# r9y9/nnmnkwii

Measured on AMD Instinct MI355X. Metric: MLPG frames/sec (batch, 60-dim mgc x3 windows), higher is better.
Workload: dtype f64

## Files before the change

nnmnkwii_amd/csrc/mlpg_strip.hip:

```cpp
#include <map>
#include <mutex>
#include <utility>
#include <limits.h>
#include <string.h>

#include "common.h"

namespace mlpg {

int launch_strip_fwd_f64(hipStream_t st, int out_dtype, const Problem &p, const WinSet &ws, void *scratch, int R, int ndg, int dgw, bool zero_ctrl);
int launch_strip_fwd_f32(hipStream_t st, int out_dtype, const Problem &p, const WinSet &ws, void *scratch, int R, int ndg, int dgw, bool zero_ctrl);
int launch_strip_bwd_f64(hipStream_t st, int out_dtype, const Problem &p, const WinSet &ws, void *scratch, int R, int ndg, int dgw, bool zero_ctrl);
int launch_strip_bwd_f32(hipStream_t st, int out_dtype, const Problem &p, const WinSet &ws, void *scratch, int R, int ndg, int dgw, bool zero_ctrl);
int launch_strip_multi_f64(hipStream_t st, const Problem &p, const WinSet &ws, void *scratch, int R, int ndg, int dgw, bool zero_ctrl, const StreamMap &sm);
int launch_strip_multi_f32(hipStream_t st, const Problem &p, const WinSet &ws, void *scratch, int R, int ndg, int dgw, bool zero_ctrl, const StreamMap &sm);
int launch_strip_tr_f64(hipStream_t st, const Problem &p, const WinSet &ws, void *scratch, int R, bool zero_ctrl, const StreamMap &sm);
int launch_strip_tr_f32(hipStream_t st, const Problem &p, const WinSet &ws, void *scratch, int R, bool zero_ctrl, const StreamMap &sm);

namespace {
#ifndef MLPG_STRIP_W
#define MLPG_STRIP_W 4
#endif
#ifndef MLPG_STRIP_M
#define MLPG_STRIP_M 16
#endif
constexpr int kStripFrames = MLPG_STRIP_M * MLPG_STRIP_W;
constexpr int kMaxStrips = 256;
constexpr int kRecBytes = 14 * 64 * 8;
constexpr int kStripNotResident = kStripMultiNotResident;
}

bool strip_supported(const Problem &p, const WinSet &ws) {
  if (p.Tmax < 1 || (p.Tmax + kStripFrames - 1) / kStripFrames > kMaxStrips) return false;
  for (int w = 0; w < ws.nw; ++w)
    if (ws.l[w] > 1 || ws.u[w] > 1) return false;
  return rows_fit_buffer(p);
}

bool strip_preferred(const Problem &p, const WinSet &ws, bool backward, int in_dtype) {
  if (!strip_supported(p, ws)) return false;
  if (p.sd >= 16 && p.Tmax > 1024) return true;
  const int ndg = (p.sd + 63) / 64, dgw = (p.sd + ndg - 1) / ndg;
  const long nitems = (long)p.B * ndg * ((p.Tmax + kStripFrames - 1) / kStripFrames);
  if (dgw < 48) return false;
  if (p.var_mode != MLPG_HIP_VAR_FRAME) return false;
  (void)backward;
  (void)in_dtype;
  return nitems >= 512;
}

bool strip_tr_supported(const Problem &p, const WinSet &ws, bool backward, int in_dtype, int out_dtype) {
  if (backward || in_dtype != out_dtype || ws.nw != 3) return false;
  if (p.sd < 1 || p.sd > 32 || p.B < 2 || !strip_supported(p, ws)) return false;
  const int u = 64 / p.sd;
  const long ld = p.ld_in > p.ld_out ? p.ld_in : p.ld_out;
  return (double)u * (double)p.Tmax * (double)ld * 8.0 < 2147483647.0;
}
bool strip_tr_preferred(const Problem &p, const WinSet &ws, bool backward, int in_dtype, int out_dtype) {
  if (!strip_tr_supported(p, ws, backward, in_dtype, out_dtype)) return false;
  const int u = 64 / p.sd;
  const long items = (long)((p.B + u - 1) / u) * ((p.Tmax + kStripFrames - 1) / kStripFrames);
  if (p.B < u) return false;
  if (p.Tmax > 1024) return items >= 64;
  return items >= (in_dtype == MLPG_HIP_F32 ? 512 : 256);
}

namespace {
std::mutex g_clean_mu;
std::map<std::pair<int, hipStream_t>, std::pair<unsigned long long, size_t>> g_clean;
void strip_scratch_forget(hipStream_t st, int device) {
  std::lock_guard<std::mutex> lk(g_clean_mu);
  g_clean[{device, st}].second = 0;
}
void *strip_scratch(hipStream_t st, int device, size_t nsg, int R, bool *zero_ctrl) {
  const size_t ctrl = (((1 + 16 + nsg) * 32 + nsg * (size_t)((R + 31) / 32 * 32)) * sizeof(int) + 255) / 256 * 256;
  unsigned long long gen = 0;
  void *sc = scratch(device, st, 3, ctrl + nsg * R * kRecBytes, &gen);
  if (!sc) return nullptr;
  *zero_ctrl = true;
  hipStreamCaptureStatus cap = hipStreamCaptureStatusNone;
  const bool capturing = hipStreamIsCapturing(st, &cap) != hipSuccess || cap != hipStreamCaptureStatusNone;
  std::lock_guard<std::mutex> lk(g_clean_mu);
  auto &c = g_clean[{device, st}];
  if (!capturing && c.first == gen && ctrl <= c.second) *zero_ctrl = false;
  c = {gen, capturing ? (size_t)0 : ctrl};
  return sc;
}
}

namespace {
__global__ void xcc_probe_kernel(int *hist) {
  if (threadIdx.x == 0) atomicAdd_system(hist + (__builtin_amdgcn_s_getreg((3 << 11) | (0 << 6) | 20) & 7), 1);
}
}
bool strip_xcd_lists_ok(hipStream_t st) {
  static std::mutex mu;
  static std::map<int, bool> seen;
  static std::map<int, int> failed;
  int dev = 0;
  if (hipGetDevice(&dev) != hipSuccess) return false;
  std::lock_guard<std::mutex> lk(mu);
  auto it = seen.find(dev);
  if (it != seen.end()) return it->second;
  hipStreamCaptureStatus cap = hipStreamCaptureStatusNone;
  if (hipStreamIsCapturing(st, &cap) != hipSuccess || cap != hipStreamCaptureStatusNone) {
    (void)hipGetLastError();
    return false;
  }
  hipStreamCaptureMode mode = hipStreamCaptureModeRelaxed;
  const bool mode_set = hipThreadExchangeStreamCaptureMode(&mode) == hipSuccess;
  bool ok = false, probed = false;
  int *h = nullptr;
  hipStream_t ps = nullptr;
  constexpr int kBlocks = 4096;
  if (hipHostMalloc((void **)&h, 8 * sizeof(int), hipHostMallocDefault) == hipSuccess) {
    for (int k = 0; k < 8; ++k) h[k] = 0;
    if (hipStreamCreateWithFlags(&ps, hipStreamNonBlocking) == hipSuccess) {
      hipLaunchKernelGGL(xcc_probe_kernel, dim3(kBlocks), dim3(64), 0, ps, h);
      if (hipGetLastError() == hipSuccess && hipStreamSynchronize(ps) == hipSuccess) {
        int lo = h[0], hi = h[0];
        for (int k = 1; k < 8; ++k) { lo = h[k] < lo ? h[k] : lo; hi = h[k] > hi ? h[k] : hi; }
        ok = lo > 0 && 2 * lo >= hi;
        probed = true;
      }
      (void)hipStreamDestroy(ps);
    }
    (void)hipHostFree(h);
  }
  (void)hipGetLastError();
  if (mode_set) (void)hipThreadExchangeStreamCaptureMode(&mode);
  if (probed) seen[dev] = ok;
  else if (++failed[dev] >= 3) seen[dev] = false;
  return ok;
}

int launch_strip_tr(hipStream_t st, int dtype, const Problem &p, const WinSet &ws, int device) {
  const int R = (p.Tmax + kStripFrames - 1) / kStripFrames;
  StreamMap sm;
  memset(&sm, 0, sizeof(sm));
  for (int q = 0; q < 4; ++q) sm.begin[q] = INT_MAX;
  sm.n = 1;
  sm.begin[0] = 0;
  sm.sd[0] = p.pitch ? p.pitch : p.sd;
  sm.tr_nd = p.sd;
  sm.tr_u = 64 / p.sd;
  sm.total = sm.tr_u * sm.tr_nd;
  sm.tr_B = p.B;
  sm.tr_in = (int)((long)p.Tmax * p.ld_in);
  sm.tr_out = (int)((long)p.Tmax * p.ld_out);
  sm.tr_stat = p.ld_status;
  const size_t nsg = (size_t)(p.B + sm.tr_u - 1) / sm.tr_u;
  bool zero_ctrl = true;
  void *sc = strip_scratch(st, device, nsg, R, &zero_ctrl);
  if (!sc) return MLPG_HIP_ENOMEM;
  const int rc = dtype == MLPG_HIP_F32 ? launch_strip_tr_f32(st, p, ws, sc, R, zero_ctrl, sm) : launch_strip_tr_f64(st, p, ws, sc, R, zero_ctrl, sm);
  if (rc == kStripNotResident) strip_scratch_forget(st, device);
  return rc;
}

int launch_strip(hipStream_t st, int dtype, int out_dtype, bool backward, const Problem &p, const WinSet &ws,
                 int device, bool try_tr) {
  if (try_tr && strip_tr_supported(p, ws, backward, dtype, out_dtype)) {
    const int rc = launch_strip_tr(st, dtype, p, ws, device);
    if (rc != kStripNotResident) return rc;
  }
  const int R = (p.Tmax + kStripFrames - 1) / kStripFrames;
  const int ndg = (p.sd + 63) / 64;
  const int dgw = (p.sd + ndg - 1) / ndg;
  const size_t nsg = (size_t)p.B * ndg;
  bool zero_ctrl = true;
  void *sc = strip_scratch(st, device, nsg, R, &zero_ctrl);
  if (!sc) return MLPG_HIP_ENOMEM;
  int rc;
  if (!backward)
    rc = dtype == MLPG_HIP_F32 ? launch_strip_fwd_f32(st, out_dtype, p, ws, sc, R, ndg, dgw, zero_ctrl)
                               : launch_strip_fwd_f64(st, out_dtype, p, ws, sc, R, ndg, dgw, zero_ctrl);
  else
    rc = dtype == MLPG_HIP_F32 ? launch_strip_bwd_f32(st, out_dtype, p, ws, sc, R, ndg, dgw, zero_ctrl)
                               : launch_strip_bwd_f64(st, out_dtype, p, ws, sc, R, ndg, dgw, zero_ctrl);
  if (rc == kStripNotResident) {
    strip_scratch_forget(st, device);
    return launch_generic(st, dtype, out_dtype, backward, p, ws, device);
  }
  return rc;
}

int launch_strip_multi(hipStream_t st, int dtype, const Problem &p, const WinSet &ws, const StreamMap &sm, int device) {
  const int R = (p.Tmax + kStripFrames - 1) / kStripFrames;
  const int ndg = (sm.total + 63) / 64;
  const int dgw = 64;
  const size_t nsg = (size_t)p.B * ndg;
  bool zero_ctrl = true;
  void *sc = strip_scratch(st, device, nsg, R, &zero_ctrl);
  if (!sc) return MLPG_HIP_ENOMEM;
  const int rc = dtype == MLPG_HIP_F32 ? launch_strip_multi_f32(st, p, ws, sc, R, ndg, dgw, zero_ctrl, sm)
                                       : launch_strip_multi_f64(st, p, ws, sc, R, ndg, dgw, zero_ctrl, sm);
  if (rc == kStripNotResident) strip_scratch_forget(st, device);
  return rc;
}

}
```

nnmnkwii_amd/csrc/mlpg_strip_bwd_f32.hip:

```cpp
#include "mlpg_strip_impl.h"
namespace mlpg {
int launch_strip_bwd_f32(hipStream_t st, int out_dtype, const Problem &p, const WinSet &ws, void *scratch, int R, int ndg, int dgw, bool zero_ctrl) {
  if (out_dtype == MLPG_HIP_F32) return strip::launch_t<float, float, true>(st, p, ws, scratch, R, ndg, dgw, zero_ctrl);
  return strip::launch_t<float, double, true>(st, p, ws, scratch, R, ndg, dgw, zero_ctrl);
}
}
```

nnmnkwii_amd/csrc/mlpg_strip_bwd_f64.hip:

```cpp
#include "mlpg_strip_impl.h"
namespace mlpg {
int launch_strip_bwd_f64(hipStream_t st, int out_dtype, const Problem &p, const WinSet &ws, void *scratch, int R, int ndg, int dgw, bool zero_ctrl) {
  if (out_dtype == MLPG_HIP_F32) return strip::launch_t<double, float, true>(st, p, ws, scratch, R, ndg, dgw, zero_ctrl);
  return strip::launch_t<double, double, true>(st, p, ws, scratch, R, ndg, dgw, zero_ctrl);
}
}
```

nnmnkwii_amd/csrc/mlpg_strip_fwd_f32.hip:

```cpp
#include "mlpg_strip_impl.h"
namespace mlpg {
int launch_strip_fwd_f32(hipStream_t st, int out_dtype, const Problem &p, const WinSet &ws, void *scratch, int R, int ndg, int dgw, bool zero_ctrl) {
  (void)out_dtype;
  return strip::launch_t<float, float, false>(st, p, ws, scratch, R, ndg, dgw, zero_ctrl);
}
}
```

nnmnkwii_amd/csrc/mlpg_strip_fwd_f64.hip:

```cpp
#include "mlpg_strip_impl.h"
namespace mlpg {
int launch_strip_fwd_f64(hipStream_t st, int out_dtype, const Problem &p, const WinSet &ws, void *scratch, int R, int ndg, int dgw, bool zero_ctrl) {
  (void)out_dtype;
  return strip::launch_t<double, double, false>(st, p, ws, scratch, R, ndg, dgw, zero_ctrl);
}
}
```

nnmnkwii_amd/csrc/mlpg_strip_impl.h:

```cpp
#pragma once
#include <stdlib.h>
#include <string.h>

#include <type_traits>

#include <mutex>
#include <vector>
#include "assemble.h"

#ifndef MLPG_STRIP_ABLATE
#define MLPG_STRIP_ABLATE 0
#endif
#ifdef MLPG_STRIP_TIMING
#define STRIP_TICK(k)                                                  \
  do {                                                                 \
    const long long t_now_ = (long long)__builtin_readcyclecounter(); \
    tq[k] += t_now_ - t_prev;                                          \
    t_prev = t_now_;                                                   \
  } while (0)
#else
#define STRIP_TICK(k) do {} while (0)
#endif

namespace mlpg {
namespace strip {

#ifndef MLPG_STRIP_W
#define MLPG_STRIP_W 4
#endif
#ifndef MLPG_STRIP_M
#define MLPG_STRIP_M 16
#endif
#ifndef MLPG_STRIP_WGS
#define MLPG_STRIP_WGS (MLPG_STRIP_W <= 4 ? 2 : 1)
#endif
constexpr int kW = MLPG_STRIP_W;
constexpr int kM = MLPG_STRIP_M;
constexpr int kN = kM - 2;
constexpr int kRec = 14;
#ifndef MLPG_STRIP_DAMP1_TOL
#define MLPG_STRIP_DAMP1_TOL 0x1p-66
#endif
#ifndef MLPG_STRIP_STAGE
#define MLPG_STRIP_STAGE (MLPG_STRIP_W > 6 ? 8 : 6)
#endif
constexpr int kStage = MLPG_STRIP_STAGE;
constexpr bool kParkOn = kM >= 16;
constexpr int kPark = kParkOn ? 2 * kN : 0;
constexpr int kFac = 10;
constexpr int kSpinLimit = 1 << 20;

enum { rT00, rT01, rT11, rH0, rH1, rD11, rD12, rD22, rF1, rF2, rL11, rL12, rL21, rL22 };

constexpr int kCtrlLine = 32;
#ifndef MLPG_STRIP_POLL_SLEEP
#define MLPG_STRIP_POLL_SLEEP 16
#endif
#ifndef MLPG_STRIP_RING_F32
#define MLPG_STRIP_RING_F32 6
#endif
#ifndef MLPG_STRIP_BWD_FRAME_MAJOR
#define MLPG_STRIP_BWD_FRAME_MAJOR 1
#endif
#ifndef MLPG_STRIP_BWD_KEEP
#define MLPG_STRIP_BWD_KEEP 1
#endif
#ifndef MLPG_STRIP_FWD_BUFSTORE
#define MLPG_STRIP_FWD_BUFSTORE 1
#endif
#ifndef MLPG_STRIP_BWD_BUFSTORE
#define MLPG_STRIP_BWD_BUFSTORE 1
#endif
#ifndef MLPG_STRIP_BWD_KARG
#define MLPG_STRIP_BWD_KARG 1
#endif
#ifndef MLPG_STRIP_FWD_KARG
#define MLPG_STRIP_FWD_KARG 1
#endif
#ifndef MLPG_STRIP_BWD_KEEP0
#define MLPG_STRIP_BWD_KEEP0 1
#endif
#ifndef MLPG_STRIP_BWD_EARLY0
#define MLPG_STRIP_BWD_EARLY0 0
#endif
#ifndef MLPG_STRIP_BWD_EARLY
#define MLPG_STRIP_BWD_EARLY 4
#endif
#ifndef MLPG_STRIP_NT_STORES
#define MLPG_STRIP_NT_STORES 1
#endif
#ifndef MLPG_STRIP_RING_F64
#define MLPG_STRIP_RING_F64 6
#endif
#ifndef MLPG_STRIP_STAGGER_DEFAULT_US
#define MLPG_STRIP_STAGGER_DEFAULT_US 0
#endif

#ifndef MLPG_STRIP_ROUTE1_TOL
#define MLPG_STRIP_ROUTE1_TOL 0x1p-66
#endif
constexpr int kMaxLists = 8;
constexpr int kLocal = 2;
constexpr double kRouteTol = 1e-11;
constexpr double kDampTol = 1e-22;
constexpr double kDamp1Tol = MLPG_STRIP_DAMP1_TOL;
struct Window { int lo, hiE, edge; };
__device__ __forceinline__ Window local_window(int r, int Ract, int k) {
  Window w;
  w.lo = r - k < 0 ? 0 : r - k;
  w.edge = r + k < Ract - 1;
  w.hiE = w.edge ? r + k : Ract - 1;
  return w;
}
struct Order { int lo, hiE, r, nt, nb, m, npos; };
__device__ __forceinline__ Order make_order(int r, int lo, int hiE) {
  Order o;
  o.lo = lo; o.hiE = hiE; o.r = r;
  o.nt = r - lo;
  o.nb = hiE - r;
  o.m = o.nt < o.nb ? o.nt : o.nb;
  o.npos = o.nt + o.nb + 1;
  return o;
}
__device__ __forceinline__ int row_of(const Order &o, int pos) {
  if (pos < 2 * o.m) return (pos & 1) ? o.hiE - (pos >> 1) : o.lo + (pos >> 1);
  if (pos < o.nt + o.nb) {
    const int k = o.m + (pos - 2 * o.m);
    return o.nt > o.nb ? o.lo + k : o.hiE - k;
  }
  return o.r;
}
__host__ __device__ inline int flag_pitch(int R) { return (R + kCtrlLine - 1) / kCtrlLine * kCtrlLine; }
__host__ __device__ inline size_t ctrl_ints(int nsg, int R) {
  return (size_t)(1 + kMaxLists + nsg) * kCtrlLine + (size_t)nsg * flag_pitch(R);
}

struct Args {
  int *ctrl;
  double *rec;
  int R;
  int ndg, dgw;
  int nsg;
  double one;
  double wc[kMaxWindows][9];
  int nlists;
  int nb, bs;
  StreamMap sm;
  int stagger;
  int wpl;
};

template <bool MULTI = false>
__device__ __forceinline__ void ticket_item(const Args &a, int tk, int lst, int &g, int &r) {
  if (MULTI) {
    g = (((tk / a.R) / a.ndg) * a.nlists + lst) * a.ndg + (tk / a.R) % a.ndg;
    r = tk % a.R;
  } else {
    const int v = (tk / a.bs) * a.nlists + lst;
    g = v / a.nb;
    r = (v - g * a.nb) * a.bs + tk % a.bs;
  }
}

struct LaneStream { int sd, din, dstat, dout, dvar; };
__device__ __forceinline__ LaneStream lane_stream_tr(const StreamMap &sm, int d) {
  const int u = d / sm.tr_nd, dl = d - u * sm.tr_nd;
  return {sm.sd[0], u * sm.tr_in + sm.in_col[0] + dl, u * sm.tr_stat + sm.stat_col[0] + dl, u * sm.tr_out + sm.out_col[0] + dl,
          sm.in_col[0] + dl};
}
__device__ __forceinline__ LaneStream lane_stream(const StreamMap &sm, int d) {
  const int s_ = (d >= sm.begin[1]) + (d >= sm.begin[2]) + (d >= sm.begin[3]);
  auto pick = [&](const int (&v)[4]) { return s_ == 0 ? v[0] : s_ == 1 ? v[1] : s_ == 2 ? v[2] : v[3]; };
  const int dl = d - pick(sm.begin);
  return {pick(sm.sd), dl + pick(sm.in_col), dl + pick(sm.stat_col), dl + pick(sm.out_col), dl + pick(sm.in_col)};
}

constexpr size_t kLdsStage = (size_t)kStage * kRec * 64 * 8;
constexpr size_t kLdsPark = (size_t)kPark * 64 * 8;
constexpr size_t kLdsFac = (size_t)(kW - 1) * kFac * 64 * 8;
constexpr size_t kLdsU = (size_t)(kW + 1) * 2 * 64 * 8;
constexpr size_t kLdsMisc = 64 + kW * 256;
constexpr size_t kLdsBytes = kLdsStage + kLdsPark + kLdsFac + kLdsU + kLdsMisc;
static_assert(kW * kRec <= kStage * kRec, "level-1 records must fit the staging area");
static_assert(kLdsBytes <= 160 * 1024 / MLPG_STRIP_WGS, "MLPG_STRIP_WGS workgroups per CU must fit the 160 KB of LDS");

__device__ __forceinline__ double fast_rcp(double d) {
  double x = __builtin_amdgcn_rcp(d);
  x = __builtin_fma(__builtin_fma(-d, x, 1.0), x, x);
  x = __builtin_fma(__builtin_fma(-d, x, 1.0), x, x);
  return x;
}
template <typename T>
__device__ __forceinline__ double tau_of(T v);
template <>
__device__ __forceinline__ double tau_of<float>(float v) {
  return (double)__fdiv_rn(1.0f, v);
}
template <>
__device__ __forceinline__ double tau_of<double>(double v) {
  return fast_rcp(v);
}

struct S2 { double a, b, c; };
struct M2 { double a, b, c, d; };
struct V2 { double x, y; };

__device__ __forceinline__ S2 sym_inv(const S2 &E, bool &bad) {
  const double det = E.a * E.c - E.b * E.b;
  bad |= (E.a <= 0.0) | (det <= 0.0) | !(det == det);
  const double idet = fast_rcp(det);
  return {E.c * idet, -E.b * idet, E.a * idet};
}
__device__ __forceinline__ M2 mul_ms(const M2 &L, const S2 &S) {
  return {L.a * S.a + L.b * S.b, L.a * S.b + L.b * S.c, L.c * S.a + L.d * S.b, L.c * S.b + L.d * S.c};
}
__device__ __forceinline__ M2 mul_sm(const S2 &S, const M2 &V) {
  return {S.a * V.a + S.b * V.c, S.a * V.b + S.b * V.d, S.b * V.a + S.c * V.c, S.b * V.b + S.c * V.d};
}
__device__ __forceinline__ M2 mul_smt(const S2 &S, const M2 &V) {
  return {S.a * V.a + S.b * V.b, S.a * V.c + S.b * V.d, S.b * V.a + S.c * V.b, S.b * V.c + S.c * V.d};
}
__device__ __forceinline__ double amax4(const M2 &m) {
  return __builtin_fmax(__builtin_fmax(__builtin_fabs(m.a), __builtin_fabs(m.b)),
                        __builtin_fmax(__builtin_fabs(m.c), __builtin_fabs(m.d)));
}
__device__ __forceinline__ M2 mul_mm(const M2 &A, const M2 &B) {
  return {A.a * B.a + A.b * B.c, A.a * B.b + A.b * B.d, A.c * B.a + A.d * B.c, A.c * B.b + A.d * B.d};
}
__device__ __forceinline__ S2 mul_mmt_sym(const M2 &A, const M2 &B) {
  return {A.a * B.a + A.b * B.b, A.a * B.c + A.b * B.d, A.c * B.c + A.d * B.d};
}
__device__ __forceinline__ S2 mul_mtm_sym(const M2 &A, const M2 &B) {
  return {A.a * B.a + A.c * B.c, A.a * B.b + A.c * B.d, A.b * B.b + A.d * B.d};
}
__device__ __forceinline__ V2 mul_mv(const M2 &A, const V2 &v) { return {A.a * v.x + A.b * v.y, A.c * v.x + A.d * v.y}; }
__device__ __forceinline__ V2 mul_mtv(const M2 &A, const V2 &v) { return {A.a * v.x + A.c * v.y, A.b * v.x + A.d * v.y}; }
__device__ __forceinline__ V2 mul_sv(const S2 &S, const V2 &v) { return {S.a * v.x + S.b * v.y, S.b * v.x + S.c * v.y}; }
__device__ __forceinline__ S2 sub(const S2 &A, const S2 &B) { return {A.a - B.a, A.b - B.b, A.c - B.c}; }
__device__ __forceinline__ S2 add(const S2 &A, const S2 &B) { return {A.a + B.a, A.b + B.b, A.c + B.c}; }
__device__ __forceinline__ V2 sub(const V2 &A, const V2 &B) { return {A.x - B.x, A.y - B.y}; }
__device__ __forceinline__ V2 add(const V2 &A, const V2 &B) { return {A.x + B.x, A.y + B.y}; }
__device__ __forceinline__ M2 neg(const M2 &A) { return {-A.a, -A.b, -A.c, -A.d}; }
__device__ __forceinline__ M2 transpose(const M2 &A) { return {A.a, A.c, A.b, A.d}; }

__device__ __forceinline__ void st_agent(double *p, double v) {
  __hip_atomic_store((unsigned long long *)p, (unsigned long long)__double_as_longlong(v), __ATOMIC_RELAXED,
                     __HIP_MEMORY_SCOPE_AGENT);
}
__device__ __forceinline__ double ld_agent(const double *p) {
  return __longlong_as_double((long long)__hip_atomic_load((const unsigned long long *)p, __ATOMIC_RELAXED,
                                                           __HIP_MEMORY_SCOPE_AGENT));
}

constexpr int kNB = kM == 16 ? 6 : 2;
constexpr int kHB = (kM + 2) / kNB;
static_assert(kHB * kNB == kM + 2, "batches must tile the 18 frames");

typedef __attribute__((ext_vector_type(2))) unsigned int u32x2;
template <typename TIN>
__device__ __forceinline__ TIN ld_row(__amdgpu_buffer_rsrc_t rs, unsigned soff, unsigned loff);
template <>
__device__ __forceinline__ double ld_row<double>(__amdgpu_buffer_rsrc_t rs, unsigned soff, unsigned loff) {
  const u32x2 v = __builtin_amdgcn_raw_buffer_load_b64(rs, loff, soff, 0);
  return __longlong_as_double((long long)(((unsigned long long)v.y << 32) | v.x));
}
template <>
__device__ __forceinline__ float ld_row<float>(__amdgpu_buffer_rsrc_t rs, unsigned soff, unsigned loff) {
  return __uint_as_float(__builtin_amdgcn_raw_buffer_load_b32(rs, loff, soff, 0));
}
template <typename TIN>
__device__ __forceinline__ TIN ld_row_g(__amdgpu_buffer_rsrc_t rs, unsigned soff, unsigned loff);
template <>
__device__ __forceinline__ double ld_row_g<double>(__amdgpu_buffer_rsrc_t rs, unsigned soff, unsigned loff) {
  const u32x2 v = __builtin_amdgcn_raw_buffer_load_b64(rs, loff, soff, 0);
  return __longlong_as_double((long long)(((unsigned long long)v.y << 32) | v.x));
}
template <>
__device__ __forceinline__ float ld_row_g<float>(__amdgpu_buffer_rsrc_t rs, unsigned soff, unsigned loff) {
  return __uint_as_float(__builtin_amdgcn_raw_buffer_load_b32(rs, loff, soff, 0));
}
__device__ __forceinline__ __amdgpu_buffer_rsrc_t make_rsrc(const void *base) {
  const unsigned long long u = (unsigned long long)base;
  const unsigned lo = __builtin_amdgcn_readfirstlane((unsigned)u), hi = __builtin_amdgcn_readfirstlane((unsigned)(u >> 32));
  return __builtin_amdgcn_make_buffer_rsrc((void *)(((unsigned long long)hi << 32) | lo), 0, 0x7fffffff, 0x00020000);
}

__device__ __forceinline__ void st_row(__amdgpu_buffer_rsrc_t rs, unsigned soff, unsigned loff, double v) {
  const unsigned long long u = (unsigned long long)__double_as_longlong(v);
  const u32x2 w = {(unsigned)u, (unsigned)(u >> 32)};
  __builtin_amdgcn_raw_buffer_store_b64(w, rs, loff, soff, MLPG_STRIP_NT_STORES ? 2 : 0);
}
__device__ __forceinline__ void st_row(__amdgpu_buffer_rsrc_t rs, unsigned soff, unsigned loff, float v) {
  __builtin_amdgcn_raw_buffer_store_b32(__float_as_uint(v), rs, loff, soff, MLPG_STRIP_NT_STORES ? 2 : 0);
}

typedef __attribute__((ext_vector_type(8))) unsigned u32x8;
typedef __attribute__((ext_vector_type(4))) unsigned u32x4;
__device__ __forceinline__ double mk_f64(unsigned lo, unsigned hi) {
  return __longlong_as_double((long long)(((unsigned long long)hi << 32) | lo));
}
template <unsigned OFF>
__device__ __forceinline__ void karg_f64x6(double (&d)[6]) {
  const unsigned long long kp = (unsigned long long)__builtin_amdgcn_kernarg_segment_ptr();
  u32x8 a;
  u32x4 b;
  asm volatile("s_load_dwordx8 %0, %2, %3\n\ts_load_dwordx4 %1, %2, %4\n\ts_waitcnt lgkmcnt(0)"
               : "=&s"(a), "=&s"(b)
               : "s"(kp), "n"(OFF), "n"(OFF + 32));
  d[0] = mk_f64(a[0], a[1]); d[1] = mk_f64(a[2], a[3]); d[2] = mk_f64(a[4], a[5]); d[3] = mk_f64(a[6], a[7]);
  d[4] = mk_f64(b[0], b[1]); d[5] = mk_f64(b[2], b[3]);
}
typedef __attribute__((ext_vector_type(16))) unsigned u32x16;
template <unsigned OFF>
__device__ __forceinline__ void karg_f64x9(double (&d)[9]) {
  const unsigned long long kp = (unsigned long long)__builtin_amdgcn_kernarg_segment_ptr();
  u32x16 a;
  u32x2 b;
  asm volatile("s_load_dwordx16 %0, %2, %3\n\ts_load_dwordx2 %1, %2, %4\n\ts_waitcnt lgkmcnt(0)"
               : "=&s"(a), "=&s"(b)
               : "s"(kp), "n"(OFF), "n"(OFF + 64));
#pragma unroll
  for (int q = 0; q < 8; ++q) d[q] = mk_f64(a[2 * q], a[2 * q + 1]);
  d[8] = mk_f64(b[0], b[1]);
}
template <unsigned OFF>
__device__ __forceinline__ void karg_f64x3(double (&d)[3]) {
  const unsigned long long kp = (unsigned long long)__builtin_amdgcn_kernarg_segment_ptr();
  u32x4 a;
  u32x2 b;
  asm volatile("s_load_dwordx4 %0, %2, %3\n\ts_load_dwordx2 %1, %2, %4\n\ts_waitcnt lgkmcnt(0)"
               : "=&s"(a), "=&s"(b)
               : "s"(kp), "n"(OFF), "n"(OFF + 16));
  d[0] = mk_f64(a[0], a[1]); d[1] = mk_f64(a[2], a[3]); d[2] = mk_f64(b[0], b[1]);
}
constexpr unsigned kKargWs = (unsigned)((sizeof(Problem) + alignof(WinSet) - 1) / alignof(WinSet) * alignof(WinSet));
constexpr unsigned kKargArgs = (unsigned)((kKargWs + sizeof(WinSet) + alignof(Args) - 1) / alignof(Args) * alignof(Args));
constexpr unsigned kKargWc = kKargArgs + (unsigned)__builtin_offsetof(Args, wc);

template <typename TIN, bool BWD, int VM, bool EDGE, int H>
__device__ __forceinline__ void load_batch(TIN (&rv)[kHB], TIN (&rm)[kHB], __amdgpu_buffer_rsrc_t mrs,
                                           __amdgpu_buffer_rsrc_t vrs, unsigned woff, unsigned loff, unsigned ldi_bytes,
                                           int f0, int lo, int hi) {
#pragma unroll
  for (int q = 0; q < kHB; ++q) {
    int t = f0 + H * kHB + q - 1;
    if (EDGE) t = t < lo ? lo : (t >= hi ? hi - 1 : t);
    const unsigned soff = (unsigned)t * ldi_bytes + woff;
    if (VM == MLPG_HIP_VAR_FRAME) rv[q] = ld_row<TIN>(vrs, soff, loff);
    if (!BWD) rm[q] = ld_row<TIN>(mrs, soff, loff);
  }
}

struct WinCoef {
  double cm, c0, cp, c00, cpp, cmm, cp0, c0m, cpm, tau_glob;
  int w;
};

template <typename TIN, bool BWD, int VM, bool EDGE, int H>
__device__ __forceinline__ void accumulate(const TIN (&rv)[kHB], const TIN (&rm)[kHB], const WinCoef &k, int f0, int lo,
                                           int hi, double (&Pd)[kM], double (&P1)[kM], double (&P2)[kM],
                                           double (&rhs)[kM], double &ca, double &cb, double &cc) {
#pragma unroll
  for (int q = 0; q < kHB; ++q) {
    const int i = H * kHB + q - 1;
    const int t = f0 + i;
    double tau = VM == MLPG_HIP_VAR_FRAME ? tau_of<TIN>(rv[q]) : k.tau_glob;
    if (MLPG_STRIP_ABLATE >= 3) {
      if (i >= 0 && i < kM) { Pd[i] += VM == MLPG_HIP_VAR_FRAME ? (double)rv[q] : 1.0; if (!BWD) rhs[i] += (double)rm[q]; }
      continue;
    }
    if (EDGE) tau *= (t >= lo && t < hi) ? 1.0 : 0.0;
    double tm = 0.0;
    if (!BWD) tm = tau * (double)rm[q];
    if (i >= 0 && i < kM) {
      Pd[i] += k.c00 * tau;
      P1[i] += k.cp0 * tau;
      if (!BWD) rhs[i] += k.c0 * tm;
    }
    if (i + 1 >= 0 && i + 1 < kM) {
      Pd[i + 1] += k.cpp * tau;
      if (!BWD) rhs[i + 1] += k.cp * tm;
    }
    if (i - 1 >= 0 && i - 1 < kM) {
      Pd[i - 1] += k.cmm * tau;
      P1[i - 1] += k.c0m * tau;
      P2[i - 1] += k.cpm * tau;
      if (!BWD) rhs[i - 1] += k.cm * tm;
    }
    if (i == -1) {
      ca += k.cpm * tau;
      cb += k.cp0 * tau;
    }
    if (i == 0) {
      cb += k.c0m * tau;
      cc += k.cpm * tau;
    }
  }
}

template <typename TIN, int VM>
__device__ __forceinline__ WinCoef win_coef(const double (*wc)[9], int w, const TIN *vglob, int sd) {
  WinCoef k;
  k.cm = wc[w][0]; k.c0 = wc[w][1]; k.cp = wc[w][2];
  k.c00 = wc[w][3]; k.cpp = wc[w][4]; k.cmm = wc[w][5];
  k.cp0 = wc[w][6]; k.c0m = wc[w][7]; k.cpm = wc[w][8];
  k.tau_glob = 1.0;
  if (VM == MLPG_HIP_VAR_GLOBAL) k.tau_glob = tau_of<TIN>(vglob[w * sd]);
  k.w = w;
  return k;
}

template <typename TIN, bool BWD, int VM, bool EDGE>
__device__ __forceinline__ void assemble(__amdgpu_buffer_rsrc_t mrs, __amdgpu_buffer_rsrc_t vrs,
                                         __amdgpu_buffer_rsrc_t grs, const TIN *__restrict__ vglob, unsigned loff,
                                         long ldi, long ldg, int sd, int f0, int T, int Tmax, const WinSet &ws,
                                         const double (*wc)[9], double (&Pd)[kM], double (&P1)[kM], double (&P2)[kM], double (&rhs)[kM],
                                         double &ca, double &cb, double &cc) {
#pragma unroll
  for (int i = 0; i < kM; ++i) Pd[i] = P1[i] = P2[i] = rhs[i] = 0.0;
  ca = cb = cc = 0.0;
  const int mw = ws.mw, nw = ws.nw;
  const unsigned ldi_bytes = (unsigned)ldi * (unsigned)sizeof(TIN), win_bytes = (unsigned)sd * (unsigned)sizeof(TIN);
  auto live_lo = [&](int w) { return w ? mw : 0; };
  auto live_hi = [&](int w) { return w ? (mw != 0 && T - mw > mw ? T - mw : mw) : T; };
  TIN rvA[kHB], rmA[kHB], rvB[kHB], rmB[kHB];
  auto clo = [&](int w) { const int l_ = live_lo(w); return l_ < T ? l_ : T - 1; };
  auto chi = [&](int w) { const int h_ = live_hi(w), l_ = clo(w); return h_ > l_ ? h_ : l_ + 1; };
  load_batch<TIN, BWD, VM, EDGE, 0>(rvA, rmA, mrs, vrs, 0u, loff, ldi_bytes, f0, clo(0), chi(0));
  if (BWD) {
#pragma unroll
    for (int i = 0; i < kM; ++i) {
      int t = f0 + i;
      if (EDGE) t = t >= T ? T - 1 : t;
      rhs[i] = (double)ld_row_g<TIN>(grs, (unsigned)t * (unsigned)ldg * (unsigned)sizeof(TIN), loff);
    }
  }
  for (int w = 0; w < nw; ++w) {
    const WinCoef k = win_coef<TIN, VM>(wc, w, vglob, sd);
    const unsigned woff = (unsigned)w * win_bytes;
    const int lo = live_lo(w), hi = live_hi(w), cl = clo(w), ch = chi(w);
#define STRIP_STEP(H, RVX, RMX, RVY, RMY)                                                                      \
    if ((H) + 1 < kNB) {                                                                                          \
    load_batch<TIN, BWD, VM, EDGE, ((H) + 1 < kNB ? (H) + 1 : 0)>(RVY, RMY, mrs, vrs, woff, loff, ldi_bytes, f0, cl, ch);             \
    __builtin_amdgcn_sched_barrier(0);                                                                          \
    accumulate<TIN, BWD, VM, EDGE, (H)>(RVX, RMX, k, f0, lo, hi, Pd, P1, P2, rhs, ca, cb, cc);                  \
    __builtin_amdgcn_sched_barrier(0);                                                                          \
    }
    STRIP_STEP(0, rvA, rmA, rvB, rmB)
    STRIP_STEP(1, rvB, rmB, rvA, rmA)
    STRIP_STEP(2, rvA, rmA, rvB, rmB)
    STRIP_STEP(3, rvB, rmB, rvA, rmA)
    STRIP_STEP(4, rvA, rmA, rvB, rmB)
#undef STRIP_STEP
    if (w + 1 < nw) load_batch<TIN, BWD, VM, EDGE, 0>(rvA, rmA, mrs, vrs, woff + win_bytes, loff, ldi_bytes, f0, clo(w + 1), chi(w + 1));
    __builtin_amdgcn_sched_barrier(0);
    accumulate<TIN, BWD, VM, EDGE, kNB - 1>(rvB, rmB, k, f0, lo, hi, Pd, P1, P2, rhs, ca, cb, cc);
    __builtin_amdgcn_sched_barrier(0);
  }
  if (EDGE) {
#pragma unroll
    for (int i = 0; i < kM; ++i) {
      const int f = f0 + i;
      if (f >= T) {
        Pd[i] = 1.0;
        P1[i] = P2[i] = rhs[i] = 0.0;
      } else {
        if (f + 1 >= T) P1[i] = 0.0;
        if (f + 2 >= T) P2[i] = 0.0;
      }
    }
    if (f0 == 0 || f0 >= T) ca = cb = cc = 0.0;
    else if (f0 + 1 >= T) cc = 0.0;
  }
}

__device__ __forceinline__ bool eliminate(double (&Pd)[kM], double (&P1)[kM], double (&P2)[kM], double (&rhs)[kM],
                                          double ca, double cb, double cc, double (&rec)[kRec]) {
  bool bad = false;
  double t00 = 0.0, t01 = 0.0, t11 = 0.0, h0 = 0.0, h1 = 0.0;
  double g1 = 0.0, g2 = 0.0, va1 = 0.0, va2 = 0.0, vb1 = 0.0, vb2 = 0.0;
  double l1p = 0.0, l2p = 0.0, l2pp = 0.0;
#pragma unroll
  for (int i = 0; i < kN; ++i) {
    const double dd = Pd[i];
    bad |= !(dd > 0.0);
    const double dinv = fast_rcp(dd);
    const double e1 = P1[i], e2 = P2[i];
    const double l1 = e1 * dinv, l2 = e2 * dinv;
    Pd[i + 1] -= l1 * e1;
    P1[i + 1] -= l2 * e1;
    Pd[i + 2] -= l2 * e2;
    const double gi = rhs[i] - l1p * g1 - l2pp * g2;
    const double ba = (i == 0) ? ca : 0.0;
    const double bb = (i == 0) ? cb : ((i == 1) ? cc : 0.0);
    const double va = ba - l1p * va1 - l2pp * va2;
    const double vb = bb - l1p * vb1 - l2pp * vb2;
    const double wa = va * dinv, wb = vb * dinv;
    t00 += wa * va;
    t01 += wa * vb;
    t11 += wb * vb;
    h0 += wa * gi;
    h1 += wb * gi;
    Pd[i] = dinv;
    P1[i] = l1;
    P2[i] = l2;
    rhs[i] = gi;
    g2 = g1; g1 = gi;
    va2 = va1; va1 = va;
    vb2 = vb1; vb1 = vb;
    l2pp = l2p; l2p = l2; l1p = l1;
    __builtin_amdgcn_sched_barrier(0);
  }
  rec[rT00] = t00; rec[rT01] = t01; rec[rT11] = t11; rec[rH0] = h0; rec[rH1] = h1;
  rec[rD11] = Pd[kN]; rec[rD12] = P1[kN]; rec[rD22] = Pd[kN + 1];
  rec[rF1] = rhs[kN] - (l1p * g1 + l2pp * g2);
  rec[rF2] = rhs[kN + 1] - l2p * g1;
  rec[rL11] = -(l1p * va1 + l2pp * va2);
  rec[rL12] = -(l1p * vb1 + l2pp * vb2);
  rec[rL21] = -(l2p * va1);
  rec[rL22] = -(l2p * vb1);
  return bad;
}

constexpr int kStd4[3][9] = {{0, 4, 0, 4, 0, 0, 0, 0, 0}, {-2, 0, 2, 0, 1, 1, 0, 0, -1}, {4, -8, 4, 16, 4, 4, -8, -8, 4}};
enum { qCm, qC0, qCp, qC00, qCpp, qCmm, qCp0, qC0m, qCpm };
constexpr int std_first(int q) { return kStd4[0][q] ? 0 : (kStd4[1][q] ? 1 : 2); }
constexpr bool std_last_has_all() {
  for (int q = 0; q < 9; ++q)
    if (kStd4[2][q] == 0) return false;
  return true;
}
static_assert(std_last_has_all(), "every entry has a window that contributes (std_first)");
__device__ __forceinline__ void std_term(double &acc, const int w, const int q, const double x, const bool init) {
  const int c4 = kStd4[w][q];
  if (c4 == 0) return;
  if (init && w == std_first(q)) acc = c4 == 4 ? x : (c4 == -4 ? -x : (0.25 * c4) * x);
  else acc = c4 == 4 ? acc + x : (c4 == -4 ? acc - x : __builtin_fma(0.25 * c4, x, acc));
}
__device__ __forceinline__ double std_apply(const int w, const double xm, const double x0, const double xp) {
  if (w == 0) return x0;
  if (w == 1) return __builtin_fma(0.5, xp, -0.5 * xm);
  return __builtin_fma(-2.0, x0, xm) + xp;
}
inline bool std_windows(const WinSet &ws, const double (*wc)[9]) {
  if (ws.nw != 3 || ws.l[0] != 0 || ws.u[0] != 0 || ws.l[1] != 1 || ws.u[1] != 1 || ws.l[2] != 1 || ws.u[2] != 1) return false;
  for (int w = 0; w < 3; ++w)
    for (int q = 0; q < 9; ++q)
      if (!(wc[w][q] == 0.25 * kStd4[w][q])) return false;
  return true;
}
inline bool stdwin_enabled() {
  static const bool on = [] { const char *e = getenv("MLPG_STRIP_STDWIN"); return !(e && *e && atoi(e) == 0); }();
  return on;
}

template <typename TIN>
struct RingDepth { static constexpr int value = MLPG_STRIP_RING_F64; };
template <>
struct RingDepth<float> { static constexpr int value = MLPG_STRIP_RING_F32; };
template <typename TIN, bool BWD, int VM, bool EDGE, int NW, bool MULTI = false, bool KEEP = false, bool LT = false, bool STD = false>
__device__ __forceinline__ bool assemble_eliminate(__amdgpu_buffer_rsrc_t mrs, __amdgpu_buffer_rsrc_t vrs,
                                                   __amdgpu_buffer_rsrc_t grs, const TIN *__restrict__ vglob,
                                                   unsigned loff, long ldi, long ldg, int sd, int f0, int T, int mw,
                                                   const double (*wc)[9], const double one, double (&Pd)[kM], double (&P1)[kM],
                                                   double (&P2)[kM], double (&rhs)[kM], double &ca, double &cb,
                                                   double &cc, double (&rec)[kRec], float (&tk)[kM + 1][NW], const int Tu = 0) {
  const unsigned ldi_bytes = (unsigned)ldi * (unsigned)sizeof(TIN), win_bytes = (unsigned)sd * (unsigned)sizeof(TIN);
  int lo[NW], hi[NW], cl[NW], ch[NW];
  int hi_l[NW];
  WinCoef k[NW];
#pragma unroll
  for (int w = 0; w < NW; ++w) {
    lo[w] = w ? mw : 0;
    hi[w] = w ? (mw != 0 && T - mw > mw ? T - mw : mw) : T;
    hi_l[w] = w ? (mw != 0 && Tu - mw > mw ? Tu - mw : mw) : Tu;
    cl[w] = lo[w] < T ? lo[w] : T - 1;
    ch[w] = hi[w] > cl[w] ? hi[w] : cl[w] + 1;
    if (STD) {
      k[w] = WinCoef{};
      k[w].tau_glob = VM == MLPG_HIP_VAR_GLOBAL ? tau_of<TIN>(vglob[w * sd]) : 1.0;
    } else {
      k[w] = win_coef<TIN, VM>(wc, w, vglob, sd);
    }
    if (VM == MLPG_HIP_VAR_UNIT) {
      double t1 = one;
      asm volatile("" : "+v"(t1));
      k[w].tau_glob = t1;
    }
  }
  constexpr int kRing = RingDepth<TIN>::value;
  TIN rv[kRing][NW], rm[kRing][NW];
  auto load_frame = [&](TIN (&v)[NW], TIN (&m)[NW], const int i) __attribute__((always_inline)) {
    unsigned frame_off = (unsigned)(f0 + i) * ldi_bytes;
    if (BWD && !EDGE) asm volatile("" : "+s"(frame_off));
#pragma unroll
    for (int w = 0; w < NW; ++w) {
      int t = f0 + i;
      if (EDGE) {
        t = t < cl[w] ? cl[w] : (t >= ch[w] ? ch[w] - 1 : t);
        frame_off = (unsigned)t * ldi_bytes;
        if (BWD) asm volatile("" : "+s"(frame_off));
      }
      const unsigned soff = MULTI ? frame_off : frame_off + (unsigned)w * win_bytes;
      const unsigned voff = MULTI ? loff + (unsigned)w * win_bytes : loff;
      if (VM == MLPG_HIP_VAR_FRAME) v[w] = ld_row<TIN>(vrs, soff, voff);
      if (!BWD) m[w] = ld_row<TIN>(mrs, soff, voff);
    }
  };
  auto accumulate_frame = [&](const TIN (&v)[NW], const TIN (&m)[NW], const int i) __attribute__((always_inline)) {
    const int t = f0 + i;
#pragma unroll
    for (int w = 0; w < NW; ++w) {
      double tau = VM == MLPG_HIP_VAR_FRAME ? tau_of<TIN>(v[w]) : k[w].tau_glob;
      double mval = BWD ? 0.0 : (double)m[w];
      if (EDGE && LT) {
        const bool lv = t >= lo[w] && t < hi_l[w];
        tau = lv ? tau : 0.0;
        mval = lv ? mval : 0.0;
      } else if (EDGE) {
        tau *= (t >= lo[w] && t < hi[w]) ? 1.0 : 0.0;
      }
      if (KEEP && i < kM) tk[i + 1][w] = (float)tau;
      double tm = 0.0;
      if (!BWD) tm = tau * mval;
      if (STD) {
        static_assert(!STD || NW == 3, "the standard set has three windows");
        if (!BWD && w != 1) asm("" : "+v"(tm));
        if (i >= 0 && i < kM) {
          std_term(Pd[i], w, qC00, tau, false);
          std_term(P1[i], w, qCp0, tau, true);
          if (!BWD) std_term(rhs[i], w, qC0, tm, false);
        }
        if (i + 1 >= 0 && i + 1 < kM) {
          std_term(Pd[i + 1], w, qCpp, tau, true);
          if (!BWD) std_term(rhs[i + 1], w, qCp, tm, true);
        }
        if (i - 1 >= 0 && i - 1 < kM) {
          std_term(Pd[i - 1], w, qCmm, tau, false);
          std_term(P1[i - 1], w, qC0m, tau, false);
          std_term(P2[i - 1], w, qCpm, tau, true);
          if (!BWD) std_term(rhs[i - 1], w, qCm, tm, false);
        }
        if (i == -1) {
          std_term(ca, w, qCpm, tau, true);
          std_term(cb, w, qCp0, tau, true);
        }
        if (i == 0) {
          std_term(cb, w, qC0m, tau, false);
          std_term(cc, w, qCpm, tau, true);
        }
        continue;
      }
      const bool first = w == 0;
      if (i >= 0 && i < kM) {
        Pd[i] += k[w].c00 * tau;
        P1[i] = first ? k[w].cp0 * tau : P1[i] + k[w].cp0 * tau;
        if (!BWD) rhs[i] += k[w].c0 * tm;
      }
      if (i + 1 >= 0 && i + 1 < kM) {
        Pd[i + 1] = first ? k[w].cpp * tau : Pd[i + 1] + k[w].cpp * tau;
        if (!BWD) rhs[i + 1] = first ? k[w].cp * tm : rhs[i + 1] + k[w].cp * tm;
      }
      if (i - 1 >= 0 && i - 1 < kM) {
        Pd[i - 1] += k[w].cmm * tau;
        P1[i - 1] += k[w].c0m * tau;
        P2[i - 1] = first ? k[w].cpm * tau : P2[i - 1] + k[w].cpm * tau;
        if (!BWD) rhs[i - 1] += k[w].cm * tm;
      }
      if (i == -1) {
        ca = first ? k[w].cpm * tau : ca + k[w].cpm * tau;
        cb = first ? k[w].cp0 * tau : cb + k[w].cp0 * tau;
      }
      if (i == 0) {
        cb += k[w].c0m * tau;
        cc = first ? k[w].cpm * tau : cc + k[w].cpm * tau;
      }
    }
  };
  auto fix_row = [&](const int i) __attribute__((always_inline)) {
    const int f = f0 + i;
    if (LT) {
      Pd[i] = f < Tu ? Pd[i] : 1.0;
      P1[i] = f + 1 < Tu ? P1[i] : 0.0;
      P2[i] = f + 2 < Tu ? P2[i] : 0.0;
      rhs[i] = f < Tu ? rhs[i] : 0.0;
      return;
    }
    const double live = f < T ? 1.0 : 0.0, live1 = f + 1 < T ? 1.0 : 0.0, live2 = f + 2 < T ? 1.0 : 0.0;
    Pd[i] = Pd[i] * live + (1.0 - live);
    P1[i] *= live1;
    P2[i] *= live2;
    rhs[i] *= live;
  };
  bool bad = false;
  double t00 = 0.0, t01 = 0.0, t11 = 0.0, h0 = 0.0, h1 = 0.0;
  double g1 = 0.0, g2 = 0.0, va1 = 0.0, va2 = 0.0, vb1 = 0.0, vb2 = 0.0;
  double l1p = 0.0, l2p = 0.0, l2pp = 0.0;
  auto elim_row = [&](const int i) __attribute__((always_inline)) {
    if (EDGE) {
      fix_row(i);
      if (i == 0 && LT) {
        const bool keep = !(f0 == 0 || f0 >= Tu), keepc = keep && !(f0 + 1 >= Tu);
        ca = keep ? ca : 0.0;
        cb = keep ? cb : 0.0;
        cc = keepc ? cc : 0.0;
      } else if (i == 0) {
        const double keep = (f0 == 0 || f0 >= T) ? 0.0 : 1.0, keepc = f0 + 1 >= T ? 0.0 : 1.0;
        ca *= keep;
        cb *= keep;
        cc *= keep * keepc;
      }
    }
    const double dd = Pd[i];
    const double dinv = fast_rcp(dd);
    if (STD) bad |= !(dinv > 0.0);
    else bad |= !(dd > 0.0);
    const double e1 = P1[i], e2 = P2[i];
    const double l1 = e1 * dinv, l2 = e2 * dinv;
    if (STD && i + 1 < kM) asm("" : "+v"(P1[i + 1]));
    Pd[i + 1] -= l1 * e1;
    P1[i + 1] -= l2 * e1;
    Pd[i + 2] -= l2 * e2;
    const double gi = rhs[i] - l1p * g1 - l2pp * g2;
    const double ba = (i == 0) ? ca : 0.0;
    const double bb = (i == 0) ? cb : ((i == 1) ? cc : 0.0);
    const double va = ba - l1p * va1 - l2pp * va2;
    const double vb = bb - l1p * vb1 - l2pp * vb2;
    const double wa = va * dinv, wb = vb * dinv;
    t00 += wa * va;
    t01 += wa * vb;
    t11 += wb * vb;
    h0 += wa * gi;
    h1 += wb * gi;
    Pd[i] = dinv;
    P1[i] = l1;
    P2[i] = l2;
    rhs[i] = gi;
    g2 = g1; g1 = gi;
    va2 = va1; va1 = va;
    vb2 = vb1; vb1 = vb;
    l2pp = l2p; l2p = l2; l1p = l1;
  };

#pragma unroll
  for (int sl = 0; sl < kRing; ++sl) load_frame(rv[sl], rm[sl], sl - 1);
  static_assert(kRing >= 2 && kRing <= kM + 2, "ring depth");
  if (BWD) {
#pragma unroll
    for (int i = 0; i < kM; ++i) {
      int t = f0 + i;
      if (EDGE) t = t >= T ? T - 1 : t;
      rhs[i] = (double)ld_row_g<TIN>(grs, (unsigned)t * (unsigned)ldg * (unsigned)sizeof(TIN), loff);
    }
  }
  __builtin_amdgcn_sched_barrier(0);
#define STRIP_SB(bit) __builtin_amdgcn_sched_barrier(0)
#define STRIP_STEP(S)                                                                   \
  if ((S) < kM + 2) {                                                                   \
  accumulate_frame(rv[(S) % kRing], rm[(S) % kRing], (S)-1);                            \
  STRIP_SB(1);                                                                          \
  if ((S) + kRing < kM + 2) { load_frame(rv[(S) % kRing], rm[(S) % kRing], (S)-1 + kRing); } \
  STRIP_SB(2);                                                                          \
  if ((S)-2 >= 0 && (S)-2 < kN) { elim_row((S)-2); }                                    \
  STRIP_SB(4);                                                                          \
  }
  STRIP_STEP(0) STRIP_STEP(1) STRIP_STEP(2) STRIP_STEP(3) STRIP_STEP(4) STRIP_STEP(5)
  STRIP_STEP(6) STRIP_STEP(7) STRIP_STEP(8) STRIP_STEP(9) STRIP_STEP(10) STRIP_STEP(11)
  STRIP_STEP(12) STRIP_STEP(13) STRIP_STEP(14) STRIP_STEP(15) STRIP_STEP(16) STRIP_STEP(17)
#undef STRIP_STEP
#undef STRIP_SB
  if (EDGE) {
    fix_row(kN);
    fix_row(kN + 1);
  }
  rec[rT00] = t00; rec[rT01] = t01; rec[rT11] = t11; rec[rH0] = h0; rec[rH1] = h1;
  rec[rD11] = Pd[kN]; rec[rD12] = P1[kN]; rec[rD22] = Pd[kN + 1];
  rec[rF1] = rhs[kN] - (l1p * g1 + l2pp * g2);
  rec[rF2] = rhs[kN + 1] - l2p * g1;
  rec[rL11] = -(l1p * va1 + l2pp * va2);
  rec[rL12] = -(l1p * vb1 + l2pp * vb2);
  rec[rL21] = -(l2p * va1);
  rec[rL22] = -(l2p * vb1);
  return bad;
}

__device__ __forceinline__ void backsub(const double (&Pd)[kM], const double (&P1)[kM], const double (&P2)[kM],
                                        double (&rhs)[kM], double ca, double cb, double cc, V2 ul, V2 u) {
  {
    double a1 = 0.0, a2 = 0.0, b1 = 0.0, b2 = 0.0, q1 = 0.0, q2 = 0.0, q3 = 0.0;
#pragma unroll
    for (int i = 0; i < kN; ++i) {
      const double ba = (i == 0) ? ca : 0.0;
      const double bb = (i == 0) ? cb : ((i == 1) ? cc : 0.0);
      const double va = ba - q1 * a1 - q3 * a2;
      const double vb = bb - q1 * b1 - q3 * b2;
      rhs[i] -= va * ul.x + vb * ul.y;
      a2 = a1; a1 = va;
      b2 = b1; b1 = vb;
      q3 = q2; q2 = P2[i]; q1 = P1[i];
    }
  }
  double x1 = u.x, x2 = u.y;
#pragma unroll
  for (int i = kN - 1; i >= 0; --i) {
    const double xi = rhs[i] * Pd[i] - P1[i] * x1 - P2[i] * x2;
    rhs[i] = xi;
    x2 = x1;
    x1 = xi;
  }
  rhs[kN] = u.x;
  rhs[kN + 1] = u.y;
}

template <typename TIN, typename TOUT, bool BWD, int VM, bool MULTI = false, bool NW3 = true, bool TR = false, bool STD = false>
__global__ __launch_bounds__(kW * 64, MLPG_STRIP_WGS) void strip_kernel(Problem p, WinSet ws, Args a) {
  static_assert(!TR || MULTI, "the transposed form is a MULTI kernel");
  static_assert(!STD || (NW3 && !MULTI), "the standard-window form: three windows, one stream");
  extern __shared__ __align__(16) unsigned char smem[];
  double *lds_rec = (double *)smem;
  double *lds_stage = (double *)smem;
  double *lds_park = (double *)(smem + kLdsStage);
  double *lds_fac = (double *)(smem + kLdsStage + kLdsPark);
  double *lds_u = (double *)(smem + kLdsStage + kLdsPark + kLdsFac);
  int *lds_misc = (int *)(smem + kLdsStage + kLdsPark + kLdsFac + kLdsU);

  const int tid = threadIdx.x, lane = tid & 63;
  const int wv = __builtin_amdgcn_readfirstlane(tid >> 6);
  if (tid < 16) lds_misc[tid] = 0;
  __syncthreads();

#ifdef MLPG_STRIP_TIMING
  long long tq[16] = {0, 0, 0, 0, 0, 0, 0, 0, 0, 0, 0, 0, 0, 0, 0, 0};
  long long t_prev = (long long)__builtin_readcyclecounter();
#endif
  const int xcd = __builtin_amdgcn_s_getreg((3 << 11) | (0 << 6) | 20) & 7;
  const int R = a.R;
  auto body = [&](const int g, const int r) __attribute__((always_inline)) {
  const int b = TR ? g * a.sm.tr_u : g / a.ndg, dg = TR ? 0 : g - b * a.ndg;
  const int Tmax = p.Tmax;
  const long ldi = p.ld_in, ldg = p.ld_gout, ldo = p.ld_out;
  int T = (p.lengths && !TR) ? p.lengths[b] : Tmax;
  T = T < 0 ? 0 : (T > Tmax ? Tmax : T);
  int Ract = (T + kW * kM - 1) / (kW * kM);
  bool xwg = MLPG_STRIP_ABLATE ? false : Ract > 1;
  const int d0 = dg * a.dgw;
  const int sd_all = MULTI ? a.sm.total : p.sd;
  const int nd = TR ? (a.sm.tr_B - b < a.sm.tr_u ? a.sm.tr_B - b : a.sm.tr_u) * a.sm.tr_nd
                    : (sd_all - d0 < a.dgw ? sd_all - d0 : a.dgw);
  const bool lane_ok = lane < nd;
  int d = d0 + (lane_ok ? lane : nd - 1);
  int Tu = T, Tmin = T;
  if (TR && p.lengths) {
    Tu = p.lengths[b + d / a.sm.tr_nd];
    Tu = Tu < 0 ? 0 : (Tu > Tmax ? Tmax : Tu);
    int tmx = Tu, tmn = Tu;
#pragma unroll
    for (int off = 32; off >= 1; off >>= 1) {
      const int o1 = __shfl_xor(tmx, off, 64), o2 = __shfl_xor(tmn, off, 64);
      tmx = o1 > tmx ? o1 : tmx;
      tmn = o2 < tmn ? o2 : tmn;
    }
    T = __builtin_amdgcn_readfirstlane(tmx);
    Tmin = __builtin_amdgcn_readfirstlane(tmn);
    Ract = (T + kW * kM - 1) / (kW * kM);
    xwg = MLPG_STRIP_ABLATE ? false : Ract > 1;
  }
  int sd = p.sd, din = d, dstat = d, dvar = d;
  if (MULTI) {
    const LaneStream ls = TR ? lane_stream_tr(a.sm, d) : lane_stream(a.sm, d);
    sd = ls.sd;
    din = ls.din;
    dstat = ls.dstat;
    dvar = ls.dvar;
    d = ls.dout;
  }
  const int f0 = (r * kW + wv) * kM;
  const int nw = NW3 ? 3 : ws.nw, mw = ws.mw;

  TOUT *out_b = (TOUT *)p.out + (size_t)b * Tmax * ldo;

  if (r >= Ract) {
    if (lane_ok) {
      for (int i = 0; i < kM; ++i) {
        const int t = f0 + i;
        if (t >= Tmax) break;
        if (!BWD) {
          out_b[(size_t)t * ldo + d] = (TOUT)0;
        } else {
          for (int w = 0; w < nw; ++w) out_b[(size_t)t * ldo + w * sd + d] = (TOUT)0;
        }
      }
    }
#if !defined(MLPG_STRIP_TIMING) && !defined(MLPG_STRIP_TRACE)
    if (r == 0 && wv == 0 && lane_ok && p.status) p.status[(size_t)b * p.ld_status + dstat] = 0;
#endif
    return;
  }

  const int dbase = MULTI ? 0 : d0;
  const unsigned loff = (unsigned)(din - dbase) * (unsigned)sizeof(TIN);
  const __amdgpu_buffer_rsrc_t mrs = make_rsrc(BWD ? (const TIN *)p.out : (const TIN *)p.mean + (size_t)b * Tmax * ldi + dbase);
  const __amdgpu_buffer_rsrc_t vrs =
      make_rsrc(VM == MLPG_HIP_VAR_FRAME ? (const TIN *)p.var + (size_t)b * Tmax * ldi + dbase : (const TIN *)p.out);
  const TIN *vglob = VM == MLPG_HIP_VAR_GLOBAL ? (const TIN *)p.var + dvar : nullptr;
  const __amdgpu_buffer_rsrc_t grs = make_rsrc(BWD ? (const TIN *)p.grad_out + (size_t)b * Tmax * ldg + d0 : (const TIN *)p.out);
  const TIN *vcol = VM == MLPG_HIP_VAR_FRAME ? (const TIN *)p.var + (size_t)b * Tmax * ldi + d : nullptr;
  (void)vcol;
#ifdef MLPG_STRIP_TIMING
  const long long t_start = (long long)__builtin_amdgcn_s_memrealtime();
#endif
  STRIP_TICK(0);
#ifdef MLPG_STRIP_TRACE
  const long long tr0 = (long long)__builtin_amdgcn_s_memrealtime();
  long long tr1 = tr0, tr2 = tr0, tra = tr0;
#endif
  double Pd[kM], P1[kM], P2[kM], rhs[kM], ca, cb, cc;
  double rec[kRec];
  bool bad = false;
  constexpr bool kKeepTau = NW3 && BWD && VM == MLPG_HIP_VAR_FRAME && (sizeof(TIN) == 4 || sizeof(TOUT) == 4) && MLPG_STRIP_BWD_KEEP && !MULTI;
  constexpr int kEpi = kM + 1;
  constexpr int kEarly = (NW3 && BWD && VM == MLPG_HIP_VAR_FRAME && sizeof(TIN) == 8 && !kKeepTau && MLPG_STRIP_BWD_FRAME_MAJOR) ? MLPG_STRIP_BWD_EARLY : 0;
  constexpr bool kSplitTail = kKeepTau && !MLPG_STRIP_BWD_KEEP0;
  constexpr int kEarly0 = kSplitTail ? MLPG_STRIP_BWD_EARLY0 : kEarly;
  static_assert(kEarly >= 0 && kEarly <= kEpi && kEarly0 >= 0 && kEarly0 <= kEpi, "MLPG_STRIP_BWD_EARLY");
  float tk[kEpi][3];
  TIN tv[kEpi][3];
  auto ldf = [&](TIN (&v)[3], const int i) __attribute__((always_inline)) {
    if (VM != MLPG_HIP_VAR_FRAME) return;
    int t = f0 + i;
    t = t < 0 ? 0 : (t >= T ? T - 1 : t);
    const unsigned ldi_b = (unsigned)ldi * (unsigned)sizeof(TIN), win_b = (unsigned)sd * (unsigned)sizeof(TIN);
#pragma unroll
    for (int w = 0; w < 3; ++w) {
      v[w] = ld_row<TIN>(vrs, (unsigned)t * ldi_b + (unsigned)w * win_b, loff);
    }
  };
  auto early_issue = [&]() __attribute__((always_inline)) {
#pragma unroll
    for (int sl = 0; sl < kEarly; ++sl) ldf(tv[sl], sl - 1);
  };
  auto early_issue0 = [&]() __attribute__((always_inline)) {
#pragma unroll
    for (int sl = 0; sl < kEarly0; ++sl) ldf(tv[sl], sl - 1);
  };
  if (f0 < T) {
    const bool interior = mw != 0 && f0 - 1 >= mw && f0 + kM < (TR ? Tmin : T) - mw;
    if (NW3 && MLPG_STRIP_ABLATE < 2) {
      double wcl[3][9];
      const double (*wcs)[9] = a.wc;
      if (!STD && BWD && MLPG_STRIP_BWD_KARG) {
        double c6[3][6];
        karg_f64x6<kKargWc + 0 * 72 + 24>(c6[0]);
        karg_f64x6<kKargWc + 1 * 72 + 24>(c6[1]);
        karg_f64x6<kKargWc + 2 * 72 + 24>(c6[2]);
#pragma unroll
        for (int w = 0; w < 3; ++w) {
          wcl[w][0] = wcl[w][1] = wcl[w][2] = 0.0;
#pragma unroll
          for (int q = 0; q < 6; ++q) wcl[w][3 + q] = c6[w][q];
        }
        wcs = wcl;
      }
      if (!STD && !BWD && MLPG_STRIP_FWD_KARG && !MULTI) {
        karg_f64x9<kKargWc + 0 * 72>(wcl[0]);
        karg_f64x9<kKargWc + 1 * 72>(wcl[1]);
        karg_f64x9<kKargWc + 2 * 72>(wcl[2]);
        wcs = wcl;
      }
      if (interior) bad = assemble_eliminate<TIN, BWD, VM, false, 3, MULTI, kKeepTau, false, STD>(mrs, vrs, grs, vglob, loff, ldi, ldg, sd, f0, T, mw, wcs, a.one, Pd, P1, P2, rhs, ca, cb, cc, rec, tk);
      else bad = assemble_eliminate<TIN, BWD, VM, true, 3, MULTI, kKeepTau, TR, STD>(mrs, vrs, grs, vglob, loff, ldi, ldg, sd, f0, T, mw, wcs, a.one, Pd, P1, P2, rhs, ca, cb, cc, rec, tk, Tu);
      STRIP_TICK(1);
#ifdef MLPG_STRIP_TRACE
      asm volatile("s_waitcnt vmcnt(0)" ::: "memory");
      tra = (long long)__builtin_amdgcn_s_memrealtime();
#endif
    } else {
    if (interior) assemble<TIN, BWD, VM, false>(mrs, vrs, grs, vglob, loff, ldi, ldg, sd, f0, T, Tmax, ws, a.wc, Pd, P1, P2, rhs, ca, cb, cc);
    else assemble<TIN, BWD, VM, true>(mrs, vrs, grs, vglob, loff, ldi, ldg, sd, f0, T, Tmax, ws, a.wc, Pd, P1, P2, rhs, ca, cb, cc);
    STRIP_TICK(1);
#ifdef MLPG_STRIP_TRACE
    asm volatile("s_waitcnt vmcnt(0)" ::: "memory");
    tra = (long long)__builtin_amdgcn_s_memrealtime();
#endif
    if (MLPG_STRIP_ABLATE < 2) bad = eliminate(Pd, P1, P2, rhs, ca, cb, cc, rec);
    else {
#pragma unroll
      for (int k = 0; k < kRec; ++k) rec[k] = Pd[k] + rhs[k];
      rec[rD11] = rec[rD22] = 1.0; rec[rD12] = 0.0;
    }
    }
  } else {
#pragma unroll
    for (int i = 0; i < kM; ++i) { Pd[i] = 1.0; P1[i] = P2[i] = rhs[i] = 0.0; }
    ca = cb = cc = 0.0;
#pragma unroll
    for (int k = 0; k < kRec; ++k) rec[k] = 0.0;
    rec[rD11] = rec[rD22] = 1.0;
    if (kKeepTau) {
#pragma unroll
      for (int i = 0; i < kEpi; ++i) tk[i][0] = tk[i][1] = tk[i][2] = 0.0f;
    }
  }
  if (bad) rec[rD11] = __builtin_nan("");
#pragma unroll
  for (int k = 0; k < kRec; ++k) lds_rec[(wv * kRec + k) * 64 + lane] = rec[k];
  if (kEarly > 0 && wv != 0) early_issue();
  STRIP_TICK(2);
  __syncthreads();
  STRIP_TICK(3);

  int timed_out = 0;
  auto tail = [&](auto use_tk_c, auto nearly_c) __attribute__((always_inline)) {
  constexpr bool kUseTk = decltype(use_tk_c)::value;
  constexpr int kNEarly = decltype(nearly_c)::value;
  STRIP_TICK(10);
  __syncthreads();
  STRIP_TICK(11);
#ifdef MLPG_STRIP_TRACE
  tr2 = (long long)__builtin_amdgcn_s_memrealtime();
#endif

  const V2 ul = {lds_u[(wv * 2) * 64 + lane], lds_u[(wv * 2 + 1) * 64 + lane]};
  const V2 uo = {lds_u[((wv + 1) * 2) * 64 + lane], lds_u[((wv + 1) * 2 + 1) * 64 + lane]};
  const double sx = lds_u[(kW * 2) * 64 + lane];
  const bool sys_bad = !(sx == sx) || !(uo.x == uo.x) || !(ul.x == ul.x);
  if (MLPG_STRIP_ABLATE < 2) backsub(Pd, P1, P2, rhs, ca, cb, cc, ul, uo);
  STRIP_TICK(12);

  if (wv == 0) {
    const int to = __builtin_amdgcn_readfirstlane(timed_out);
    const unsigned long long m = to ? ~0ull : __ballot(sys_bad && lane_ok);
    if (m != 0ull && lane == 0) {
      int *line = a.ctrl + (1 + kMaxLists + g) * kCtrlLine;
      __hip_atomic_fetch_or(line + 2, (int)(unsigned)m, __ATOMIC_RELAXED, __HIP_MEMORY_SCOPE_AGENT);
      __hip_atomic_fetch_or(line + 3, (int)(unsigned)(m >> 32), __ATOMIC_RELAXED, __HIP_MEMORY_SCOPE_AGENT);
      if (to) __hip_atomic_store(line + 4, 1, __ATOMIC_RELAXED, __HIP_MEMORY_SCOPE_AGENT);
    }
#if !defined(MLPG_STRIP_TIMING) && !defined(MLPG_STRIP_TRACE)
    if (r == 0 && lane_ok && p.status) p.status[(size_t)b * p.ld_status + dstat] = 0;
#endif
  }
  const bool zero_out = sys_bad || timed_out;

#ifndef MLPG_STRIP_TIMING
  if (!lane_ok) return;
#endif
  if (!BWD) {
#if MLPG_STRIP_FWD_BUFSTORE
    const __amdgpu_buffer_rsrc_t ors_f = make_rsrc(out_b);
    const unsigned ooff_f = (unsigned)d * (unsigned)sizeof(TOUT), ldo_b = (unsigned)ldo * (unsigned)sizeof(TOUT);
#pragma unroll
    for (int i = 0; i < kM; ++i) {
      const int t = f0 + i;
      if (t < Tmax) st_row(ors_f, (unsigned)t * ldo_b, ooff_f, (t < T && !zero_out) ? (TOUT)rhs[i] : (TOUT)0);
    }
#else
#pragma unroll
    for (int i = 0; i < kM; ++i) {
      const int t = f0 + i;
#if MLPG_STRIP_NT_STORES
      if (t < Tmax) __builtin_nontemporal_store((t < T && !zero_out) ? (TOUT)rhs[i] : (TOUT)0, &out_b[(size_t)t * ldo + d]);
#else
      if (t < Tmax) out_b[(size_t)t * ldo + d] = (t < T && !zero_out) ? (TOUT)rhs[i] : (TOUT)0;
#endif
    }
#endif
  } else {
    const unsigned ldi_bytes = (unsigned)ldi * (unsigned)sizeof(TIN), win_bytes = (unsigned)sd * (unsigned)sizeof(TIN);
    auto load_w = [&](TIN (&v)[kM + 1], const int w) __attribute__((always_inline)) {
      if (VM != MLPG_HIP_VAR_FRAME) return;
#pragma unroll
      for (int i = -1; i < kM; ++i) {
        int t = f0 + i;
        t = t < 0 ? 0 : (t >= T ? T - 1 : t);
        v[i + 1] = ld_row<TIN>(vrs, (unsigned)t * ldi_bytes + (unsigned)w * win_bytes, loff);
      }
    };
    auto emit_w = [&](const TIN (&v)[kM + 1], const int w) __attribute__((always_inline)) {
      const double cm = a.wc[w][0], c0 = a.wc[w][1], cp = a.wc[w][2];
      double tau_glob = 1.0;
      if (VM == MLPG_HIP_VAR_GLOBAL) tau_glob = tau_of<TIN>(vglob[w * sd]);
      TOUT *ow = out_b + (size_t)w * sd + d;
#pragma unroll
      for (int i = -1; i < kM; ++i) {
        const int t = f0 + i;
        if (t < 0 || t >= Tmax) continue;
        if (t >= T) {
          if (i >= 0) ow[(size_t)t * ldo] = (TOUT)0;
          continue;
        }
        if (i == -1 && f0 >= T) continue;
        if (i == kM - 1 && t != T - 1) continue;
        const bool lv = w ? (mw != 0 && t >= mw && t < T - mw) : true;
        double tau = 0.0;
        if (lv) tau = VM == MLPG_HIP_VAR_FRAME ? tau_of<TIN>(v[i + 1]) : tau_glob;
        const double xm = (i == -1) ? ul.x : ((i == 0) ? ul.y : rhs[i > 0 ? i - 1 : 0]);
        const double x0 = (i == -1) ? ul.y : rhs[i >= 0 ? i : 0];
        const double xp = (i == kM - 1) ? 0.0 : rhs[i + 1];
        const double gval = tau * (cm * xm + c0 * x0 + cp * xp);
        ow[(size_t)t * ldo] = zero_out ? (TOUT)0 : (TOUT)gval;
      }
    };
    if (MLPG_STRIP_BWD_FRAME_MAJOR && NW3) {
      double tg[3] = {1.0, 1.0, 1.0};
      if (VM == MLPG_HIP_VAR_GLOBAL) {
#pragma unroll
        for (int w = 0; w < 3; ++w) tg[w] = tau_of<TIN>(vglob[w * sd]);
      }
      const __amdgpu_buffer_rsrc_t ors_e = make_rsrc(out_b);
      const unsigned ooff_e = (unsigned)d * (unsigned)sizeof(TOUT);
      (void)ors_e; (void)ooff_e;
      double we[3][3] = {};
      if (STD) {
      } else if (MLPG_STRIP_BWD_KARG) {
        karg_f64x3<kKargWc + 0 * 72>(we[0]);
        karg_f64x3<kKargWc + 1 * 72>(we[1]);
        karg_f64x3<kKargWc + 2 * 72>(we[2]);
      } else {
#pragma unroll
        for (int w = 0; w < 3; ++w) { we[w][0] = a.wc[w][0]; we[w][1] = a.wc[w][1]; we[w][2] = a.wc[w][2]; }
      }
      auto emitf = [&](const int sl) __attribute__((always_inline)) {
        const int i = sl - 1;
        const int t = f0 + i;
        if (t < 0 || t >= Tmax) return;
        TOUT *orow = out_b + (size_t)t * ldo + d;
        unsigned row_off = (unsigned)t * (unsigned)ldo * (unsigned)sizeof(TOUT);
        if (MLPG_STRIP_BWD_BUFSTORE) asm volatile("" : "+s"(row_off));
        auto put = [&](const int w, const TOUT val) __attribute__((always_inline)) {
#if MLPG_STRIP_BWD_BUFSTORE
          st_row(ors_e, row_off + (unsigned)w * (unsigned)sd * (unsigned)sizeof(TOUT), ooff_e, val);
          return;
#endif
#if MLPG_STRIP_NT_STORES
          __builtin_nontemporal_store(val, orow + (size_t)w * sd);
#else
          orow[(size_t)w * sd] = val;
#endif
        };
        if (t >= T) {
          if (i >= 0) { put(0, (TOUT)0); put(1, (TOUT)0); put(2, (TOUT)0); }
          return;
        }
        if (i == -1 && f0 >= T) return;
        if (i == kM - 1 && t != T - 1) return;
        const double xm = (i == -1) ? ul.x : ((i == 0) ? ul.y : rhs[i > 0 ? i - 1 : 0]);
        const double x0 = (i == -1) ? ul.y : rhs[i >= 0 ? i : 0];
        const double xp = (i == kM - 1) ? 0.0 : rhs[i + 1];
#pragma unroll
        for (int w = 0; w < 3; ++w) {
          const bool lv = w ? (mw != 0 && t >= mw && t < T - mw) : true;
          double tau = 0.0;
          if (kUseTk) {
            float tf = tk[sl][w];
            asm volatile("" : "+v"(tf));
            tau = (double)tf;
          }
          else if (lv) tau = VM == MLPG_HIP_VAR_FRAME ? tau_of<TIN>(tv[sl][w]) : tg[w];
          const double gval = STD ? tau * std_apply(w, xm, x0, xp) : tau * (we[w][0] * xm + we[w][1] * x0 + we[w][2] * xp);
          put(w, zero_out ? (TOUT)0 : (TOUT)gval);
        }
      };
      if (!kUseTk) {
#pragma unroll
        for (int sl = kNEarly; sl < kEpi; ++sl) ldf(tv[sl], sl - 1);
      }
      __builtin_amdgcn_sched_barrier(0);
#define STRIP_EPI(S)                                                        \
      if ((S) < kEpi) {                                                       \
      emitf((S));                                                             \
      __builtin_amdgcn_sched_barrier(0);                                      \
      }
      STRIP_EPI(0) STRIP_EPI(1) STRIP_EPI(2) STRIP_EPI(3) STRIP_EPI(4) STRIP_EPI(5) STRIP_EPI(6) STRIP_EPI(7) STRIP_EPI(8)
      STRIP_EPI(9) STRIP_EPI(10) STRIP_EPI(11) STRIP_EPI(12) STRIP_EPI(13) STRIP_EPI(14) STRIP_EPI(15) STRIP_EPI(16)
#undef STRIP_EPI
    } else {
    TIN tvA[kM + 1], tvB[kM + 1];
      load_w(tvA, 0);
      for (int w = 0; w < nw; w += 2) {
        if (w + 1 < nw) load_w(tvB, w + 1);
        __builtin_amdgcn_sched_barrier(0);
        emit_w(tvA, w);
        __builtin_amdgcn_sched_barrier(0);
        if (w + 1 < nw) {
          if (w + 2 < nw) load_w(tvA, w + 2);
          __builtin_amdgcn_sched_barrier(0);
          emit_w(tvB, w + 1);
          __builtin_amdgcn_sched_barrier(0);
        }
      }
    }
    }
#ifdef MLPG_STRIP_TIMING
  asm volatile("s_waitcnt vmcnt(0)" ::: "memory");
  STRIP_TICK(13);
  if (wv == 0 && lane == 0 && p.status && b < 8 && r < 16 && dg == 0)
  {
    for (int k = 0; k < 16; ++k) p.status[(b * 16 + r) * 16 + k] = (int)tq[k];
  }
#endif
#ifdef MLPG_STRIP_TRACE
  if (wv == 0 && lane == 0 && p.status && (g * R + r) * 4 + 3 < p.B * p.ld_status) {
    int *tp = p.status + (g * R + r) * 4;
    tp[0] = (int)(tr0 & 0x3FFFFFFF); tp[1] = (int)(tra - tr0) | ((int)(tr1 - tr0) << 16); tp[2] = (int)(tr2 - tr0);
    tp[3] = (int)((long long)__builtin_amdgcn_s_memrealtime() - tr0) | (xcd << 24);
  }
#endif
  };
  if (wv == 0) {
    if (kParkOn) {
#pragma unroll
      for (int i = 0; i < kN; ++i) {
        lds_park[i * 64 + lane] = rhs[i];
        lds_park[(kN + i) * 64 + lane] = P2[i];
      }
    }
    S2 E_s = {1.0, 0.0, 1.0};
    V2 g_s = {0.0, 0.0};
    auto R_ = [&](int j, int k) __attribute__((always_inline)) { return lds_rec[(j * kRec + k) * 64 + lane]; };
    S2 E = {R_(0, rD11), R_(0, rD12), R_(0, rD22)};
    V2 gg = {R_(0, rF1), R_(0, rF2)};
    M2 V = {R_(0, rL11), R_(0, rL12), R_(0, rL21), R_(0, rL22)};
    if (r == 0) V = {0.0, 0.0, 0.0, 0.0};
    S2 Ts = {R_(0, rT00), R_(0, rT01), R_(0, rT11)};
    V2 hs = {R_(0, rH0), R_(0, rH1)};
    if (kW > 1) {
      E = sub(E, S2{R_(1, rT00), R_(1, rT01), R_(1, rT11)});
      gg = sub(gg, V2{R_(1, rH0), R_(1, rH1)});
    }
    bool bad2 = false;
#pragma unroll
    for (int j = 0; j + 1 < kW; ++j) {
      const S2 Einv = sym_inv(E, bad2);
      const M2 L = {R_(j + 1, rL11), R_(j + 1, rL12), R_(j + 1, rL21), R_(j + 1, rL22)};
      const M2 Mn = mul_ms(L, Einv);
      const M2 EV = mul_sm(Einv, V);
      const V2 c = mul_sv(Einv, gg);
      Ts = add(Ts, mul_mtm_sym(V, EV));
      hs = add(hs, mul_mtv(V, c));
      double *f = lds_fac + (size_t)j * kFac * 64 + lane;
      f[0 * 64] = c.x; f[1 * 64] = c.y;
      f[2 * 64] = EV.a; f[3 * 64] = EV.b; f[4 * 64] = EV.c; f[5 * 64] = EV.d;
      f[6 * 64] = Mn.a; f[7 * 64] = Mn.b; f[8 * 64] = Mn.c; f[9 * 64] = Mn.d;
      S2 Dn = {R_(j + 1, rD11), R_(j + 1, rD12), R_(j + 1, rD22)};
      V2 Fn = {R_(j + 1, rF1), R_(j + 1, rF2)};
      if (j + 2 < kW) {
        Dn = sub(Dn, S2{R_(j + 2, rT00), R_(j + 2, rT01), R_(j + 2, rT11)});
        Fn = sub(Fn, V2{R_(j + 2, rH0), R_(j + 2, rH1)});
      }
      E = sub(Dn, mul_mmt_sym(Mn, L));
      gg = sub(Fn, mul_mv(Mn, gg));
      V = neg(mul_mm(Mn, V));
      __builtin_amdgcn_sched_barrier(0);
    }
    if (bad2) E.a = __builtin_nan("");
    E_s = E;
    g_s = gg;
    STRIP_TICK(4);
    int route = kLocal;
    if (xwg) {
      double *rp = a.rec + ((size_t)g * R + r) * (kRec * 64) + lane;
      st_agent(rp + 0 * 64, E.a); st_agent(rp + 1 * 64, E.b); st_agent(rp + 2 * 64, E.c);
      st_agent(rp + 3 * 64, gg.x); st_agent(rp + 4 * 64, gg.y);
      st_agent(rp + 5 * 64, V.a); st_agent(rp + 6 * 64, V.b); st_agent(rp + 7 * 64, V.c); st_agent(rp + 8 * 64, V.d);
      st_agent(rp + 9 * 64, Ts.a); st_agent(rp + 10 * 64, Ts.b); st_agent(rp + 11 * 64, Ts.c);
      st_agent(rp + 12 * 64, hs.x); st_agent(rp + 13 * 64, hs.y);
      {
        bool badr = false;
        const double t_own = 2.0 * amax4(mul_sm(sym_inv(E, badr), V));
        auto any_over = [&](const double tol) { return __ballot(lane_ok && !(t_own <= tol)) != 0ull; };
        route = !any_over(MLPG_STRIP_ROUTE1_TOL) ? 1 : !any_over(kRouteTol) ? kLocal : !any_over(3e-6) ? 4 : !any_over(1.8e-3) ? 8 : !any_over(4.2e-2) ? 16 : 0;
        if (2 * route + 1 >= Ract) route = route > kLocal ? 0 : route;
        if (lane == 0) lds_misc[3] = route;
      }
      const int kwin = route ? route : kLocal;
      if (route && route <= kLocal && 2 * route + 1 <= kStage) {
        const Window w = local_window(r, Ract, route);
        const Order o = make_order(r, w.lo, w.hiE);
        const double own[kRec] = {E.a, E.b, E.c, gg.x, gg.y, V.a, V.b, V.c, V.d, Ts.a, Ts.b, Ts.c, hs.x, hs.y};
#pragma unroll
        for (int k = 0; k < kRec; ++k) lds_stage[((o.npos - 1) * kRec + k) * 64 + lane] = own[k];
      }
      asm volatile("s_waitcnt vmcnt(0)" ::: "memory");
      STRIP_TICK(5);
      int *cnt = a.ctrl + (1 + kMaxLists + g) * kCtrlLine;
      int *flags = a.ctrl + (1 + kMaxLists + a.nsg) * kCtrlLine + (size_t)g * flag_pitch(R);
      if (lane == 0) {
        __hip_atomic_fetch_add(cnt, 1, __ATOMIC_RELAXED, __HIP_MEMORY_SCOPE_AGENT);
        __hip_atomic_store(flags + r, 1, __ATOMIC_RELAXED, __HIP_MEMORY_SCOPE_AGENT);
      }
      {
        const Window w = local_window(r, Ract, kwin);
        int spins = 0, ok = 1;
        for (;;) {
          int f = 1;
          if (route == 0) f = __hip_atomic_load(cnt, __ATOMIC_RELAXED, __HIP_MEMORY_SCOPE_AGENT) >= Ract;
          else if (lane <= w.hiE - w.lo) f = __hip_atomic_load(flags + w.lo + lane, __ATOMIC_RELAXED, __HIP_MEMORY_SCOPE_AGENT);
          if (__ballot(f == 0) == 0ull) break;
          __builtin_amdgcn_s_sleep(MLPG_STRIP_POLL_SLEEP);
          if (++spins > kSpinLimit) { ok = 0; break; }
        }
        if (lane == 0) {
          if (!ok) atomicAdd(a.ctrl, 1);
          lds_misc[1] = ok;
        }
      }
      STRIP_TICK(6);
    }
    __syncthreads();
    STRIP_TICK(7);
#ifdef MLPG_STRIP_TRACE
    tr1 = (long long)__builtin_amdgcn_s_memrealtime();
#endif
    V2 sig = {0.0, 0.0}, sprev = {0.0, 0.0};
    if (xwg) {
      timed_out = !__builtin_amdgcn_readfirstlane(lds_misc[1]);
      double damp = 0.0;
      auto sweep = [&](const int lo, const int hiE, const int edge) __attribute__((always_inline)) {
        const Order o = make_order(r, lo, hiE);
        S2 Ainv = {0.0, 0.0, 0.0};
        V2 av = {0.0, 0.0};
        M2 Mn = {0.0, 0.0, 0.0, 0.0};
        S2 Sb = {0.0, 0.0, 0.0}, Tn = {0.0, 0.0, 0.0};
        V2 sb = {0.0, 0.0}, hn = {0.0, 0.0};
        M2 Vn = {0.0, 0.0, 0.0, 0.0};
        double dt = lo > 0 ? 1.0 : 0.0, db = edge ? 1.0 : 0.0;
        bool bad3 = false;
        S2 Ej = {0.0, 0.0, 0.0};
        V2 gj = {0.0, 0.0};
        M2 Vj = {0.0, 0.0, 0.0, 0.0};
        struct Rec { S2 E; V2 g; M2 V; S2 T; V2 h; };
        auto rd = [&](const int q) __attribute__((always_inline)) {
          double c[kRec];
#pragma unroll
          for (int kk = 0; kk < kRec; ++kk) c[kk] = lds_stage[(q * kRec + kk) * 64 + lane];
          return Rec{{c[0], c[1], c[2]}, {c[3], c[4]}, {c[5], c[6], c[7], c[8]}, {c[9], c[10], c[11]}, {c[12], c[13]}};
        };
        auto top_finalize = [&](const Rec &k) __attribute__((always_inline)) {
          const S2 A = sub(sub(Ej, k.T), mul_mmt_sym(Mn, Vj));
          const V2 aa = sub(sub(gj, k.h), mul_mv(Mn, av));
          Ainv = sym_inv(A, bad3);
          av = aa;
          Mn = mul_ms(k.V, Ainv);
          dt *= 2.0 * amax4(mul_sm(Ainv, Vj));
        };
        auto top_pend = [&](const Rec &k) __attribute__((always_inline)) { Ej = k.E; gj = k.g; Vj = k.V; };
        auto bot_edge = [&](const Rec &k) __attribute__((always_inline)) { Tn = k.T; hn = k.h; Vn = k.V; };
        auto bot_row = [&](const Rec &k) __attribute__((always_inline)) {
          const S2 B = sub(sub(k.E, Tn), Sb);
          const V2 bv = sub(sub(k.g, hn), sb);
          const S2 Binv = sym_inv(B, bad3);
          db *= 2.0 * amax4(mul_smt(Binv, Vn));
          const M2 Wm = mul_sm(Binv, k.V);
          Sb = mul_mtm_sym(k.V, Wm);
          sb = mul_mtv(k.V, mul_sv(Binv, bv));
          Tn = k.T; hn = k.h; Vn = k.V;
        };
        for (int p0 = 0; p0 < o.npos; p0 += kStage) {
          const int kn = o.npos - p0 < kStage ? o.npos - p0 : kStage;
          __syncthreads();
          STRIP_TICK(8);
          if (!timed_out) {
#ifndef MLPG_L3_NOPRIO
            __builtin_amdgcn_s_setprio(2);
#endif
            int q = 0;
            while (q < kn) {
              const int pos = p0 + q;
              if (pos < 2 * o.m) {
                const int idx = pos >> 1;
                const Rec kt = rd(q), kb = rd(q + 1);
                if (idx == 0) {
                  top_pend(kt);
                  if (edge) bot_edge(kb);
                  else bot_row(kb);
                } else {
                  top_finalize(kt);
                  bot_row(kb);
                  top_pend(kt);
                }
                q += 2;
              } else if (pos < o.nt + o.nb) {
                const int idx = o.m + (pos - 2 * o.m);
                const Rec k = rd(q);
                if (o.nt > o.nb) {
                  if (idx > 0) top_finalize(k);
                  top_pend(k);
                } else {
                  if (idx == 0 && edge) bot_edge(k);
                  else bot_row(k);
                }
                q += 1;
              } else {
                const Rec k = rd(q);
                if (o.nt > 0) top_finalize(k);
                S2 B = sub(sub(k.E, Tn), Sb);
                V2 bv = sub(sub(k.g, hn), sb);
                if (o.nt > 0) {
                  B = sub(B, mul_mmt_sym(Mn, k.V));
                  bv = sub(bv, mul_mv(Mn, av));
                }
                const S2 Binv = sym_inv(B, bad3);
                sig = mul_sv(Binv, bv);
                sprev = {0.0, 0.0};
                db *= 2.0 * amax4(mul_smt(Binv, Vn));
                if (o.nt > 0) {
                  sprev = sub(mul_sv(Ainv, av), mul_mtv(Mn, sig));
                  dt *= __builtin_fmax(1.0, 2.0 * amax4(mul_sm(Binv, k.V)));
                  db *= __builtin_fmax(1.0, 2.0 * amax4(mul_smt(Ainv, k.V)));
                }
                if (bad3) sig.x = __builtin_nan("");
                q += 1;
              }
            }
            __builtin_amdgcn_s_setprio(0);
          }
          STRIP_TICK(9);
          __syncthreads();
        }
        damp = dt > db ? dt : db;
      };
      if (route == 0) {
        sweep(0, Ract - 1, 0);
      } else {
        int cur = route;
        int *cnt = a.ctrl + (1 + kMaxLists + g) * kCtrlLine;
        int *flags = a.ctrl + (1 + kMaxLists + a.nsg) * kCtrlLine + (size_t)g * flag_pitch(R);
        for (;;) {
          const Window w = local_window(r, Ract, cur);
          const bool full_range = w.lo == 0 && !w.edge;
          sweep(w.lo, w.hiE, w.edge);
          const double tolw = cur == 1 ? kDamp1Tol : kDampTol;
          const bool lane_fine = !lane_ok || full_range || (damp < tolw && sig.x == sig.x);
          const int accept = timed_out || __ballot(!lane_fine) == 0ull;
          const int next = accept ? 0 : ((cur == 1 && kLocal > 1) ? 1 : 2);
          int ok = 1;
          if (next == 1) {
            const Window w2 = local_window(r, Ract, kLocal);
            int spins = 0;
            for (;;) {
              int f = 1;
              if (lane <= w2.hiE - w2.lo) f = __hip_atomic_load(flags + w2.lo + lane, __ATOMIC_RELAXED, __HIP_MEMORY_SCOPE_AGENT);
              if (__ballot(f == 0) == 0ull) break;
              __builtin_amdgcn_s_sleep(MLPG_STRIP_POLL_SLEEP);
              if (++spins > kSpinLimit) { ok = 0; break; }
            }
          } else if (next == 2) {
            int spins = 0;
            while (__hip_atomic_load(cnt, __ATOMIC_RELAXED, __HIP_MEMORY_SCOPE_AGENT) < Ract) {
              __builtin_amdgcn_s_sleep(32);
              if (++spins > kSpinLimit) { ok = 0; break; }
            }
          }
          if (lane == 0) {
            if (!ok) atomicAdd(a.ctrl, 1);
            if (next) lds_misc[1] = ok;
            lds_misc[2] = next;
          }
          __syncthreads();
          if (next == 0) break;
          timed_out = !ok;
          if (next == 2) {
            sweep(0, Ract - 1, 0);
            break;
          }
          cur = kLocal;
        }
      }
    } else {
      bool bad3 = false;
      const S2 Ai = sym_inv(E_s, bad3);
      sig = mul_sv(Ai, g_s);
      if (bad3) sig.x = __builtin_nan("");
    }

    if (kEarly0 > 0) early_issue0();
    double *up = lds_u + lane;
    up[0] = sprev.x; up[64] = sprev.y;
    up[(kW * 2) * 64] = sig.x; up[(kW * 2 + 1) * 64] = sig.y;
    V2 un = sig;
#pragma unroll
    for (int j = kW - 2; j >= 0; --j) {
      const double *f = lds_fac + (size_t)j * kFac * 64 + lane;
      const V2 c = {f[0 * 64], f[1 * 64]};
      const M2 EV = {f[2 * 64], f[3 * 64], f[4 * 64], f[5 * 64]};
      const M2 Mn = {f[6 * 64], f[7 * 64], f[8 * 64], f[9 * 64]};
      const V2 uj = sub(sub(c, mul_mv(EV, sprev)), mul_mtv(Mn, un));
      up[((j + 1) * 2) * 64] = uj.x; up[((j + 1) * 2 + 1) * 64] = uj.y;
      un = uj;
    }
    if (kParkOn) {
#pragma unroll
      for (int i = 0; i < kN; ++i) {
        rhs[i] = lds_park[i * 64 + lane];
        P2[i] = lds_park[(kN + i) * 64 + lane];
      }
    }
    if (kSplitTail) tail(std::integral_constant<bool, kKeepTau && MLPG_STRIP_BWD_KEEP0>{}, std::integral_constant<int, kEarly0>{});
  } else {
    __syncthreads();
    if (xwg) {
      timed_out = !__builtin_amdgcn_readfirstlane(lds_misc[1]);
      constexpr int kSlots = (kStage + kW - 2) / (kW - 1);
      double sv[kSlots][kRec];
      bool own_slot[kSlots];
      bool skip_own = true;
      auto stage_load = [&](int lo, int hi, int p0, int kn) __attribute__((always_inline)) {
        const Order o = make_order(r, lo, hi);
#pragma unroll
        for (int sl = 0; sl < kSlots; ++sl) {
          const int q = (wv - 1) + sl * (kW - 1);
          const int pos = p0 + q;
          const int row_ = row_of(o, pos);
          own_slot[sl] = skip_own && pos == o.npos - 1;
          if (q < kn && !timed_out && !own_slot[sl]) {
            const int row = row_;
            const double *rp = a.rec + ((size_t)g * R + row) * (kRec * 64) + lane;
#pragma unroll
            for (int k = 0; k < kRec; ++k) sv[sl][k] = ld_agent(rp + k * 64);
          }
        }
      };
      auto stage = [&](const int lo, const int hi) __attribute__((always_inline)) {
        const int npos = hi - lo + 1;
        stage_load(lo, hi, 0, npos < kStage ? npos : kStage);
        for (int p0 = 0; p0 < npos; p0 += kStage) {
          const int kn = npos - p0 < kStage ? npos - p0 : kStage;
#pragma unroll
          for (int sl = 0; sl < kSlots; ++sl) {
            const int q = (wv - 1) + sl * (kW - 1);
            if (q < kn && !timed_out && !own_slot[sl]) {
#pragma unroll
              for (int k = 0; k < kRec; ++k) lds_stage[(q * kRec + k) * 64 + lane] = sv[sl][k];
            }
          }
          __syncthreads();
          if (p0 + kStage < npos) stage_load(lo, hi, p0 + kStage, npos - p0 - kStage < kStage ? npos - p0 - kStage : kStage);
          __syncthreads();
        }
      };
      const int route = __builtin_amdgcn_readfirstlane(lds_misc[3]);
      if (route == 0) {
        skip_own = false;
        stage(0, Ract - 1);
      } else {
        skip_own = route <= kLocal && 2 * route + 1 <= kStage;
        int cur = route;
        for (;;) {
          const Window w = local_window(r, Ract, cur);
          stage(w.lo, w.hiE);
          __syncthreads();
          const int next = __builtin_amdgcn_readfirstlane(lds_misc[2]);
          if (next == 0) break;
          timed_out = !__builtin_amdgcn_readfirstlane(lds_misc[1]);
          skip_own = false;
          if (next == 2) {
            stage(0, Ract - 1);
            break;
          }
          cur = kLocal;
        }
      }
    }
    if (kSplitTail) tail(std::integral_constant<bool, kKeepTau>{}, std::integral_constant<int, kEarly>{});
  }
  if (!kSplitTail) tail(std::false_type{}, std::integral_constant<int, kEarly>{});
  };

  bool first_item = true;
  const long long t_launch = (long long)__builtin_amdgcn_s_memrealtime();
  for (int k = 0; k < a.nlists; ++k) {
    const int lst = (xcd + k) % a.nlists;
    const int lim = MULTI ? ((a.nsg / a.ndg - lst + a.nlists - 1) / a.nlists) * a.ndg * R
                          : ((a.nsg * a.nb - lst + a.nlists - 1) / a.nlists) * a.bs;
    int *ticket = a.ctrl + (1 + lst) * kCtrlLine;
    for (;;) {
      if (tid == 0) {
        int tk = lim;
        if (__hip_atomic_load(ticket, __ATOMIC_RELAXED, __HIP_MEMORY_SCOPE_AGENT) < lim) tk = atomicAdd(ticket, 1);
        if (first_item && a.stagger > 0 && tk < a.wpl && tk < lim) {
          const long long until = t_launch + (long long)tk * a.stagger / a.wpl;
          while ((long long)__builtin_amdgcn_s_memrealtime() < until) __builtin_amdgcn_s_sleep(8);
        }
        lds_misc[0] = tk;
      }
      first_item = false;
      __syncthreads();
      const int tk = __builtin_amdgcn_readfirstlane(lds_misc[0]);
      if (tk >= lim) break;
#ifdef MLPG_STRIP_TIMING
      t_prev = (long long)__builtin_readcyclecounter();
      for (int q = 0; q < 16; ++q) tq[q] = 0;
#endif
      int g_it, r_it;
      ticket_item<MULTI>(a, tk, lst, g_it, r_it);
      if (r_it < R) body(g_it, r_it);
      __syncthreads();
    }
    __syncthreads();
  }
}

template <typename TIN, typename TOUT, bool BWD, bool MULTI = false, bool TR = false>
__global__ void __launch_bounds__(256) verdict_kernel(const Problem p, const WinSet ws, const Args a) {
  const int lane = threadIdx.x & 63;
  const int g = blockIdx.x * 4 + (threadIdx.x >> 6);
  if (g >= a.nsg) return;
  int *line = a.ctrl + (1 + kMaxLists + g) * kCtrlLine;
  const unsigned long long m = (unsigned long long)(unsigned)line[2] | ((unsigned long long)(unsigned)line[3] << 32);
  const int timed_out = line[4];
  __builtin_amdgcn_wave_barrier();
  if (lane < 5) line[lane] = 0;
  for (int i = lane; i < flag_pitch(a.R); i += 64) a.ctrl[(1 + kMaxLists + a.nsg) * kCtrlLine + (size_t)g * flag_pitch(a.R) + i] = 0;
  if (g == 0)
    for (int i = lane; i < (1 + kMaxLists) * kCtrlLine; i += 64) a.ctrl[i] = 0;
  if (m == 0ull) return;
  const int b = TR ? g * a.sm.tr_u : g / a.ndg, dg = TR ? 0 : g - b * a.ndg;
  const int d0 = dg * a.dgw;
  const int sd_all = MULTI ? a.sm.total : p.sd;
  const int nd = TR ? (a.sm.tr_B - b < a.sm.tr_u ? a.sm.tr_B - b : a.sm.tr_u) * a.sm.tr_nd
                    : (sd_all - d0 < a.dgw ? sd_all - d0 : a.dgw);
  if (lane >= nd || !((m >> lane) & 1ull)) return;
  int d = d0 + lane, dstat = d;
  const int Tmax = p.Tmax;
  int T = p.lengths ? p.lengths[TR ? b + d / a.sm.tr_nd : b] : Tmax;
  T = T < 0 ? 0 : (T > Tmax ? Tmax : T);
  int status = -1;
  if (MULTI) {
    const LaneStream ls = TR ? lane_stream_tr(a.sm, d) : lane_stream(a.sm, d);
    Problem q = p;
    q.sd = ls.sd;
    q.D = ws.nw * ls.sd;
    q.mean = (const TIN *)p.mean + ls.din;
    q.var = p.var ? (const void *)((const TIN *)p.var + (p.var_mode == MLPG_HIP_VAR_GLOBAL ? ls.dvar : ls.din)) : nullptr;
    if (!timed_out) {
      const SysView<TIN, BWD> view = make_view<TIN, BWD>(q, ws, b, 0, T);
      status = first_bad_pivot<2, TIN, BWD>(view, ws);
      if (status == 0) status = -2;
    }
    dstat = ls.dstat;
    d = ls.dout;
  } else if (!timed_out) {
    const SysView<TIN, BWD> view = make_view<TIN, BWD>(p, ws, b, d, T);
    status = first_bad_pivot<2, TIN, BWD>(view, ws);
    if (status == 0) status = -2;
  }
  if (p.status) p.status[(size_t)b * p.ld_status + dstat] = status;
  TOUT *out_b = (TOUT *)p.out + (size_t)b * Tmax * p.ld_out;
  for (int t = 0; t < Tmax; ++t) {
    if (!BWD) out_b[(size_t)t * p.ld_out + d] = (TOUT)0;
    else
      for (int w = 0; w < ws.nw; ++w) out_b[(size_t)t * p.ld_out + w * p.sd + d] = (TOUT)0;
  }
}

inline size_t ctrl_bytes(int nsg, int R) { return (ctrl_ints(nsg, R) * sizeof(int) + 255) / 256 * 256; }

constexpr int kNotResident = -1000;

inline int resident_grid(const void *kern, int threads, size_t lds, int *out) {
  struct Entry { const void *kern; int dev, grid; };
  static std::mutex mu;
  static std::vector<Entry> cache;
  int dev = 0;
  MLPG_HIP_CHECK(hipGetDevice(&dev));
  {
    std::lock_guard<std::mutex> lk(mu);
    for (const Entry &e : cache)
      if (e.kern == kern && e.dev == dev) { *out = e.grid; return 0; }
  }
  int ncu = 0, per_cu = 0;
  MLPG_HIP_CHECK(hipFuncSetAttribute(kern, hipFuncAttributeMaxDynamicSharedMemorySize, (int)lds));
  MLPG_HIP_CHECK(hipDeviceGetAttribute(&ncu, hipDeviceAttributeMultiprocessorCount, dev));
  MLPG_HIP_CHECK(hipOccupancyMaxActiveBlocksPerMultiprocessor(&per_cu, kern, threads, lds));
  if (ncu < 1 || per_cu < 1) {
    set_error("strip kernel: occupancy query returned %d workgroups per CU on %d CUs", per_cu, ncu);
    return MLPG_HIP_ERUNTIME;
  }
  std::lock_guard<std::mutex> lk(mu);
  cache.push_back({kern, dev, ncu * per_cu});
  *out = ncu * per_cu;
  return 0;
}

template <typename TIN, typename TOUT, bool BWD>
constexpr bool kHasStd = !(BWD && sizeof(TIN) == 8 && sizeof(TOUT) == 8);
typedef void (*KernelFn)(Problem, WinSet, Args);
template <typename TIN, typename TOUT, bool BWD>
KernelFn std_kernel();
template <> KernelFn std_kernel<double, double, false>();
template <> KernelFn std_kernel<float, float, false>();
template <> KernelFn std_kernel<double, float, true>();
template <> KernelFn std_kernel<float, float, true>();
template <> KernelFn std_kernel<float, double, true>();
#define MLPG_STRIP_STD_KERNEL(TIN, TOUT, BWD) \
  template <> KernelFn std_kernel<TIN, TOUT, BWD>() { return strip_kernel<TIN, TOUT, BWD, MLPG_HIP_VAR_FRAME, false, true, false, true>; }

template <typename TIN, typename TOUT, bool BWD, bool MULTI, bool TR = false>
int launch_impl(hipStream_t st, const Problem &p, const WinSet &ws, void *scratch_base, int R, int ndg, int dgw,
                bool zero_ctrl, const StreamMap *smap) {
  Args a;
  memset(&a.sm, 0, sizeof(a.sm));
  if (MULTI) a.sm = *smap;
  const int nsg = TR ? (p.B + smap->tr_u - 1) / smap->tr_u : p.B * ndg;
  a.ctrl = (int *)scratch_base;
  a.rec = (double *)((char *)scratch_base + ctrl_bytes(nsg, R));
  a.R = R;
  a.ndg = ndg;
  a.dgw = dgw;
  a.nsg = nsg;
  a.one = 1.0;
  for (int w = 0; w < ws.nw; ++w) {
    const int l = ws.l[w], u = ws.u[w];
    const double *cw = ws.c + ws.off[w];
    const double cm = l ? cw[0] : 0.0, c0 = cw[l], cp = u ? cw[l + 1] : 0.0;
    const double v[9] = {cm, c0, cp, c0 * c0, cp * cp, cm * cm, cp * c0, c0 * cm, cp * cm};
    for (int q = 0; q < 9; ++q) a.wc[w][q] = v[q];
  }
  const long nitems = (long)nsg * R;
  auto go = [&](auto kern) -> int {
    int resident = 0;
    if (int rc = resident_grid((const void *)kern, kW * 64, kLdsBytes, &resident)) return rc;
    const int cap = resident / (2 * kMaxLists);
    a.nb = 1;
    a.bs = R;
    a.nlists = 1;
    if (nitems >= 512 && cap >= 1 && (R <= cap || (!MULTI && strip_xcd_lists_ok(st)))) {
      a.nlists = kMaxLists;
      a.nb = (R + cap - 1) / cap;
      a.bs = (R + a.nb - 1) / a.nb;
    }
    if (nitems > resident && R > resident / 2) return kNotResident;
    if (zero_ctrl) MLPG_HIP_CHECK(hipMemsetAsync(a.ctrl, 0, ctrl_ints(nsg, R) * sizeof(int), st));
    long grid = nitems < resident ? nitems : resident;
    {
      static const long capg = [] { const char *e = getenv("MLPG_STRIP_GRID_CAP"); return e ? atol(e) : 0L; }();
      if (capg >= 16 * kMaxLists && capg < grid && R <= capg / (2 * kMaxLists)) grid = capg;
    }
    a.stagger = 0;
    a.wpl = (int)(grid / a.nlists);
    {
      static const double us = [] { const char *e = getenv("MLPG_STRIP_STAGGER_US"); return e ? atof(e) : (double)MLPG_STRIP_STAGGER_DEFAULT_US; }();
      if (us > 0 && a.wpl >= 2 && nitems >= 3 * grid) a.stagger = (int)(us * 100.0);
    }
    note_launch(TR ? kCountStripTr : MULTI ? kCountStripMulti : kCountStrip);
    hipLaunchKernelGGL(kern, dim3((unsigned)grid), dim3(kW * 64), kLdsBytes, st, p, ws, a);
    MLPG_HIP_CHECK(hipGetLastError());
    hipLaunchKernelGGL((verdict_kernel<TIN, TOUT, BWD, MULTI, TR>), dim3((unsigned)((nsg + 3) / 4)), dim3(256), 0, st, p, ws, a);
    MLPG_HIP_CHECK(hipGetLastError());
    return 0;
  };
  if constexpr (MULTI) {
    if constexpr (TR) {
      if (p.var_mode == MLPG_HIP_VAR_GLOBAL) return go(strip_kernel<TIN, TOUT, false, MLPG_HIP_VAR_GLOBAL, true, true, true>);
      if (p.var_mode == MLPG_HIP_VAR_UNIT) return go(strip_kernel<TIN, TOUT, false, MLPG_HIP_VAR_UNIT, true, true, true>);
    }
    return go(strip_kernel<TIN, TOUT, false, MLPG_HIP_VAR_FRAME, true, true, TR>);
  } else {
    if (ws.nw == 3) {
      if constexpr (kHasStd<TIN, TOUT, BWD>) {
        if (p.var_mode == MLPG_HIP_VAR_FRAME && std_windows(ws, a.wc) && stdwin_enabled()) return go(std_kernel<TIN, TOUT, BWD>());
      }
      switch (p.var_mode) {
        case MLPG_HIP_VAR_FRAME: return go(strip_kernel<TIN, TOUT, BWD, MLPG_HIP_VAR_FRAME, false, true>);
        case MLPG_HIP_VAR_GLOBAL: return go(strip_kernel<TIN, TOUT, BWD, MLPG_HIP_VAR_GLOBAL, false, true>);
        default: return go(strip_kernel<TIN, TOUT, BWD, MLPG_HIP_VAR_UNIT, false, true>);
      }
    }
    switch (p.var_mode) {
      case MLPG_HIP_VAR_FRAME: return go(strip_kernel<TIN, TOUT, BWD, MLPG_HIP_VAR_FRAME, false, false>);
      case MLPG_HIP_VAR_GLOBAL: return go(strip_kernel<TIN, TOUT, BWD, MLPG_HIP_VAR_GLOBAL, false, false>);
      default: return go(strip_kernel<TIN, TOUT, BWD, MLPG_HIP_VAR_UNIT, false, false>);
    }
  }
}

template <typename TIN, typename TOUT, bool BWD>
int launch_t(hipStream_t st, const Problem &p, const WinSet &ws, void *scratch_base, int R, int ndg, int dgw,
             bool zero_ctrl) {
  return launch_impl<TIN, TOUT, BWD, false>(st, p, ws, scratch_base, R, ndg, dgw, zero_ctrl, nullptr);
}
template <typename TIN, typename TOUT>
int launch_multi_t(hipStream_t st, const Problem &p, const WinSet &ws, void *scratch_base, int R, int ndg, int dgw,
                   bool zero_ctrl, const StreamMap &smap) {
  return launch_impl<TIN, TOUT, false, true>(st, p, ws, scratch_base, R, ndg, dgw, zero_ctrl, &smap);
}
template <typename TIN, typename TOUT>
int launch_tr_t(hipStream_t st, const Problem &p, const WinSet &ws, void *scratch_base, int R, bool zero_ctrl, const StreamMap &smap) {
  return launch_impl<TIN, TOUT, false, true, true>(st, p, ws, scratch_base, R, 1, 64, zero_ctrl, &smap);
}

}
}
```

nnmnkwii_amd/csrc/mlpg_strip_multi_f32.hip:

```cpp
#include "mlpg_strip_impl.h"
namespace mlpg {
int launch_strip_multi_f32(hipStream_t st, const Problem &p, const WinSet &ws, void *scratch, int R, int ndg, int dgw, bool zero_ctrl, const StreamMap &sm) {
  return strip::launch_multi_t<float, float>(st, p, ws, scratch, R, ndg, dgw, zero_ctrl, sm);
}
int launch_strip_tr_f32(hipStream_t st, const Problem &p, const WinSet &ws, void *scratch, int R, bool zero_ctrl, const StreamMap &sm) {
  return strip::launch_tr_t<float, float>(st, p, ws, scratch, R, zero_ctrl, sm);
}
}
```

nnmnkwii_amd/csrc/mlpg_strip_multi_f64.hip:

```cpp
#include "mlpg_strip_impl.h"
namespace mlpg {
int launch_strip_multi_f64(hipStream_t st, const Problem &p, const WinSet &ws, void *scratch, int R, int ndg, int dgw, bool zero_ctrl, const StreamMap &sm) {
  return strip::launch_multi_t<double, double>(st, p, ws, scratch, R, ndg, dgw, zero_ctrl, sm);
}
int launch_strip_tr_f64(hipStream_t st, const Problem &p, const WinSet &ws, void *scratch, int R, bool zero_ctrl, const StreamMap &sm) {
  return strip::launch_tr_t<double, double>(st, p, ws, scratch, R, zero_ctrl, sm);
}
}
```

Before: 1.283 billion.

## Use epoch-tagged strip flags instead of clearing them in the verdict pass

```diff
diff --git a/nnmnkwii_amd/csrc/mlpg_strip.hip b/nnmnkwii_amd/csrc/mlpg_strip.hip
--- a/nnmnkwii_amd/csrc/mlpg_strip.hip
+++ b/nnmnkwii_amd/csrc/mlpg_strip.hip
@@ -2,20 +2,21 @@
 #include <mutex>
 #include <utility>
 #include <limits.h>
+#include <stdint.h>
 #include <string.h>
 
 #include "common.h"
 
 namespace mlpg {
 
-int launch_strip_fwd_f64(hipStream_t st, int out_dtype, const Problem &p, const WinSet &ws, void *scratch, int R, int ndg, int dgw, bool zero_ctrl);
-int launch_strip_fwd_f32(hipStream_t st, int out_dtype, const Problem &p, const WinSet &ws, void *scratch, int R, int ndg, int dgw, bool zero_ctrl);
-int launch_strip_bwd_f64(hipStream_t st, int out_dtype, const Problem &p, const WinSet &ws, void *scratch, int R, int ndg, int dgw, bool zero_ctrl);
-int launch_strip_bwd_f32(hipStream_t st, int out_dtype, const Problem &p, const WinSet &ws, void *scratch, int R, int ndg, int dgw, bool zero_ctrl);
-int launch_strip_multi_f64(hipStream_t st, const Problem &p, const WinSet &ws, void *scratch, int R, int ndg, int dgw, bool zero_ctrl, const StreamMap &sm);
-int launch_strip_multi_f32(hipStream_t st, const Problem &p, const WinSet &ws, void *scratch, int R, int ndg, int dgw, bool zero_ctrl, const StreamMap &sm);
-int launch_strip_tr_f64(hipStream_t st, const Problem &p, const WinSet &ws, void *scratch, int R, bool zero_ctrl, const StreamMap &sm);
-int launch_strip_tr_f32(hipStream_t st, const Problem &p, const WinSet &ws, void *scratch, int R, bool zero_ctrl, const StreamMap &sm);
+int launch_strip_fwd_f64(hipStream_t st, int out_dtype, const Problem &p, const WinSet &ws, void *scratch, int R, int ndg, int dgw, bool zero_ctrl, int epoch);
+int launch_strip_fwd_f32(hipStream_t st, int out_dtype, const Problem &p, const WinSet &ws, void *scratch, int R, int ndg, int dgw, bool zero_ctrl, int epoch);
+int launch_strip_bwd_f64(hipStream_t st, int out_dtype, const Problem &p, const WinSet &ws, void *scratch, int R, int ndg, int dgw, bool zero_ctrl, int epoch);
+int launch_strip_bwd_f32(hipStream_t st, int out_dtype, const Problem &p, const WinSet &ws, void *scratch, int R, int ndg, int dgw, bool zero_ctrl, int epoch);
+int launch_strip_multi_f64(hipStream_t st, const Problem &p, const WinSet &ws, void *scratch, int R, int ndg, int dgw, bool zero_ctrl, int epoch, const StreamMap &sm);
+int launch_strip_multi_f32(hipStream_t st, const Problem &p, const WinSet &ws, void *scratch, int R, int ndg, int dgw, bool zero_ctrl, int epoch, const StreamMap &sm);
+int launch_strip_tr_f64(hipStream_t st, const Problem &p, const WinSet &ws, void *scratch, int R, bool zero_ctrl, int epoch, const StreamMap &sm);
+int launch_strip_tr_f32(hipStream_t st, const Problem &p, const WinSet &ws, void *scratch, int R, bool zero_ctrl, int epoch, const StreamMap &sm);
 
 namespace {
 #ifndef MLPG_STRIP_W
@@ -67,12 +68,20 @@
 
 namespace {
 std::mutex g_clean_mu;
-std::map<std::pair<int, hipStream_t>, std::pair<unsigned long long, size_t>> g_clean;
+struct Clean {
+  unsigned long long gen = 0;
+  size_t ctrl = 0;
+  size_t nsg = 0;
+  size_t cap_nsg = SIZE_MAX;
+  size_t cap_ctrl = SIZE_MAX;
+  int epoch = 0;
+};
+std::map<std::pair<int, hipStream_t>, Clean> g_clean;
 void strip_scratch_forget(hipStream_t st, int device) {
   std::lock_guard<std::mutex> lk(g_clean_mu);
-  g_clean[{device, st}].second = 0;
-}
-void *strip_scratch(hipStream_t st, int device, size_t nsg, int R, bool *zero_ctrl) {
+  g_clean[{device, st}].ctrl = 0;
+}
+void *strip_scratch(hipStream_t st, int device, size_t nsg, int R, bool *zero_ctrl, int *epoch) {
   const size_t ctrl = (((1 + 16 + nsg) * 32 + nsg * (size_t)((R + 31) / 32 * 32)) * sizeof(int) + 255) / 256 * 256;
   unsigned long long gen = 0;
   void *sc = scratch(device, st, 3, ctrl + nsg * R * kRecBytes, &gen);
@@ -81,9 +90,22 @@
   hipStreamCaptureStatus cap = hipStreamCaptureStatusNone;
   const bool capturing = hipStreamIsCapturing(st, &cap) != hipSuccess || cap != hipStreamCaptureStatusNone;
   std::lock_guard<std::mutex> lk(g_clean_mu);
-  auto &c = g_clean[{device, st}];
-  if (!capturing && c.first == gen && ctrl <= c.second) *zero_ctrl = false;
-  c = {gen, capturing ? (size_t)0 : ctrl};
+  Clean &c = g_clean[{device, st}];
+  if (c.gen != gen) c = Clean{};
+  const bool wrap = c.epoch >= INT_MAX - 1;
+  if (wrap) {
+    c.epoch = 0;
+    if (c.cap_nsg != SIZE_MAX) c.cap_ctrl = 0;
+  }
+  if (!capturing && !wrap && c.ctrl != 0 && ctrl <= c.ctrl && nsg <= c.nsg && nsg <= c.cap_nsg && ctrl <= c.cap_ctrl) *zero_ctrl = false;
+  if (capturing) {
+    if (nsg < c.cap_nsg) c.cap_nsg = nsg;
+    if (ctrl < c.cap_ctrl) c.cap_ctrl = ctrl;
+  }
+  c.gen = gen;
+  c.ctrl = capturing ? (size_t)0 : ctrl;
+  c.nsg = nsg;
+  *epoch = ++c.epoch;
   return sc;
 }
 }
@@ -151,9 +173,10 @@
   sm.tr_stat = p.ld_status;
   const size_t nsg = (size_t)(p.B + sm.tr_u - 1) / sm.tr_u;
   bool zero_ctrl = true;
-  void *sc = strip_scratch(st, device, nsg, R, &zero_ctrl);
+  int epoch = 0;
+  void *sc = strip_scratch(st, device, nsg, R, &zero_ctrl, &epoch);
   if (!sc) return MLPG_HIP_ENOMEM;
-  const int rc = dtype == MLPG_HIP_F32 ? launch_strip_tr_f32(st, p, ws, sc, R, zero_ctrl, sm) : launch_strip_tr_f64(st, p, ws, sc, R, zero_ctrl, sm);
+  const int rc = dtype == MLPG_HIP_F32 ? launch_strip_tr_f32(st, p, ws, sc, R, zero_ctrl, epoch, sm) : launch_strip_tr_f64(st, p, ws, sc, R, zero_ctrl, epoch, sm);
   if (rc == kStripNotResident) strip_scratch_forget(st, device);
   return rc;
 }
@@ -169,15 +192,16 @@
   const int dgw = (p.sd + ndg - 1) / ndg;
   const size_t nsg = (size_t)p.B * ndg;
   bool zero_ctrl = true;
-  void *sc = strip_scratch(st, device, nsg, R, &zero_ctrl);
+  int epoch = 0;
+  void *sc = strip_scratch(st, device, nsg, R, &zero_ctrl, &epoch);
   if (!sc) return MLPG_HIP_ENOMEM;
   int rc;
   if (!backward)
-    rc = dtype == MLPG_HIP_F32 ? launch_strip_fwd_f32(st, out_dtype, p, ws, sc, R, ndg, dgw, zero_ctrl)
-                               : launch_strip_fwd_f64(st, out_dtype, p, ws, sc, R, ndg, dgw, zero_ctrl);
+    rc = dtype == MLPG_HIP_F32 ? launch_strip_fwd_f32(st, out_dtype, p, ws, sc, R, ndg, dgw, zero_ctrl, epoch)
+                               : launch_strip_fwd_f64(st, out_dtype, p, ws, sc, R, ndg, dgw, zero_ctrl, epoch);
   else
-    rc = dtype == MLPG_HIP_F32 ? launch_strip_bwd_f32(st, out_dtype, p, ws, sc, R, ndg, dgw, zero_ctrl)
-                               : launch_strip_bwd_f64(st, out_dtype, p, ws, sc, R, ndg, dgw, zero_ctrl);
+    rc = dtype == MLPG_HIP_F32 ? launch_strip_bwd_f32(st, out_dtype, p, ws, sc, R, ndg, dgw, zero_ctrl, epoch)
+                               : launch_strip_bwd_f64(st, out_dtype, p, ws, sc, R, ndg, dgw, zero_ctrl, epoch);
   if (rc == kStripNotResident) {
     strip_scratch_forget(st, device);
     return launch_generic(st, dtype, out_dtype, backward, p, ws, device);
@@ -191,10 +215,11 @@
   const int dgw = 64;
   const size_t nsg = (size_t)p.B * ndg;
   bool zero_ctrl = true;
-  void *sc = strip_scratch(st, device, nsg, R, &zero_ctrl);
+  int epoch = 0;
+  void *sc = strip_scratch(st, device, nsg, R, &zero_ctrl, &epoch);
   if (!sc) return MLPG_HIP_ENOMEM;
-  const int rc = dtype == MLPG_HIP_F32 ? launch_strip_multi_f32(st, p, ws, sc, R, ndg, dgw, zero_ctrl, sm)
-                                       : launch_strip_multi_f64(st, p, ws, sc, R, ndg, dgw, zero_ctrl, sm);
+  const int rc = dtype == MLPG_HIP_F32 ? launch_strip_multi_f32(st, p, ws, sc, R, ndg, dgw, zero_ctrl, epoch, sm)
+                                       : launch_strip_multi_f64(st, p, ws, sc, R, ndg, dgw, zero_ctrl, epoch, sm);
   if (rc == kStripNotResident) strip_scratch_forget(st, device);
   return rc;
 }
diff --git a/nnmnkwii_amd/csrc/mlpg_strip_bwd_f32.hip b/nnmnkwii_amd/csrc/mlpg_strip_bwd_f32.hip
--- a/nnmnkwii_amd/csrc/mlpg_strip_bwd_f32.hip
+++ b/nnmnkwii_amd/csrc/mlpg_strip_bwd_f32.hip
@@ -1,7 +1,7 @@
 #include "mlpg_strip_impl.h"
 namespace mlpg {
-int launch_strip_bwd_f32(hipStream_t st, int out_dtype, const Problem &p, const WinSet &ws, void *scratch, int R, int ndg, int dgw, bool zero_ctrl) {
-  if (out_dtype == MLPG_HIP_F32) return strip::launch_t<float, float, true>(st, p, ws, scratch, R, ndg, dgw, zero_ctrl);
-  return strip::launch_t<float, double, true>(st, p, ws, scratch, R, ndg, dgw, zero_ctrl);
+int launch_strip_bwd_f32(hipStream_t st, int out_dtype, const Problem &p, const WinSet &ws, void *scratch, int R, int ndg, int dgw, bool zero_ctrl, int epoch) {
+  if (out_dtype == MLPG_HIP_F32) return strip::launch_t<float, float, true>(st, p, ws, scratch, R, ndg, dgw, zero_ctrl, epoch);
+  return strip::launch_t<float, double, true>(st, p, ws, scratch, R, ndg, dgw, zero_ctrl, epoch);
 }
 }
diff --git a/nnmnkwii_amd/csrc/mlpg_strip_bwd_f64.hip b/nnmnkwii_amd/csrc/mlpg_strip_bwd_f64.hip
--- a/nnmnkwii_amd/csrc/mlpg_strip_bwd_f64.hip
+++ b/nnmnkwii_amd/csrc/mlpg_strip_bwd_f64.hip
@@ -1,7 +1,7 @@
 #include "mlpg_strip_impl.h"
 namespace mlpg {
-int launch_strip_bwd_f64(hipStream_t st, int out_dtype, const Problem &p, const WinSet &ws, void *scratch, int R, int ndg, int dgw, bool zero_ctrl) {
-  if (out_dtype == MLPG_HIP_F32) return strip::launch_t<double, float, true>(st, p, ws, scratch, R, ndg, dgw, zero_ctrl);
-  return strip::launch_t<double, double, true>(st, p, ws, scratch, R, ndg, dgw, zero_ctrl);
+int launch_strip_bwd_f64(hipStream_t st, int out_dtype, const Problem &p, const WinSet &ws, void *scratch, int R, int ndg, int dgw, bool zero_ctrl, int epoch) {
+  if (out_dtype == MLPG_HIP_F32) return strip::launch_t<double, float, true>(st, p, ws, scratch, R, ndg, dgw, zero_ctrl, epoch);
+  return strip::launch_t<double, double, true>(st, p, ws, scratch, R, ndg, dgw, zero_ctrl, epoch);
 }
 }
diff --git a/nnmnkwii_amd/csrc/mlpg_strip_fwd_f32.hip b/nnmnkwii_amd/csrc/mlpg_strip_fwd_f32.hip
--- a/nnmnkwii_amd/csrc/mlpg_strip_fwd_f32.hip
+++ b/nnmnkwii_amd/csrc/mlpg_strip_fwd_f32.hip
@@ -1,7 +1,7 @@
 #include "mlpg_strip_impl.h"
 namespace mlpg {
-int launch_strip_fwd_f32(hipStream_t st, int out_dtype, const Problem &p, const WinSet &ws, void *scratch, int R, int ndg, int dgw, bool zero_ctrl) {
+int launch_strip_fwd_f32(hipStream_t st, int out_dtype, const Problem &p, const WinSet &ws, void *scratch, int R, int ndg, int dgw, bool zero_ctrl, int epoch) {
   (void)out_dtype;
-  return strip::launch_t<float, float, false>(st, p, ws, scratch, R, ndg, dgw, zero_ctrl);
+  return strip::launch_t<float, float, false>(st, p, ws, scratch, R, ndg, dgw, zero_ctrl, epoch);
 }
 }
diff --git a/nnmnkwii_amd/csrc/mlpg_strip_fwd_f64.hip b/nnmnkwii_amd/csrc/mlpg_strip_fwd_f64.hip
--- a/nnmnkwii_amd/csrc/mlpg_strip_fwd_f64.hip
+++ b/nnmnkwii_amd/csrc/mlpg_strip_fwd_f64.hip
@@ -1,7 +1,7 @@
 #include "mlpg_strip_impl.h"
 namespace mlpg {
-int launch_strip_fwd_f64(hipStream_t st, int out_dtype, const Problem &p, const WinSet &ws, void *scratch, int R, int ndg, int dgw, bool zero_ctrl) {
+int launch_strip_fwd_f64(hipStream_t st, int out_dtype, const Problem &p, const WinSet &ws, void *scratch, int R, int ndg, int dgw, bool zero_ctrl, int epoch) {
   (void)out_dtype;
-  return strip::launch_t<double, double, false>(st, p, ws, scratch, R, ndg, dgw, zero_ctrl);
+  return strip::launch_t<double, double, false>(st, p, ws, scratch, R, ndg, dgw, zero_ctrl, epoch);
 }
 }
diff --git a/nnmnkwii_amd/csrc/mlpg_strip_impl.h b/nnmnkwii_amd/csrc/mlpg_strip_impl.h
--- a/nnmnkwii_amd/csrc/mlpg_strip_impl.h
+++ b/nnmnkwii_amd/csrc/mlpg_strip_impl.h
@@ -53,6 +53,8 @@
 enum { rT00, rT01, rT11, rH0, rH1, rD11, rD12, rD22, rF1, rF2, rL11, rL12, rL21, rL22 };
 
 constexpr int kCtrlLine = 32;
+constexpr int kDoneWord = 1;
+constexpr int kDoneMarked = 1 << 30;
 #ifndef MLPG_STRIP_POLL_SLEEP
 #define MLPG_STRIP_POLL_SLEEP 16
 #endif
@@ -96,6 +98,9 @@
 #define MLPG_STRIP_STAGGER_DEFAULT_US 0
 #endif
 
+#ifndef MLPG_STRIP_SETTLE_INLINE
+#define MLPG_STRIP_SETTLE_INLINE 0
+#endif
 #ifndef MLPG_STRIP_ROUTE1_TOL
 #define MLPG_STRIP_ROUTE1_TOL 0x1p-66
 #endif
@@ -148,6 +153,7 @@
   StreamMap sm;
   int stagger;
   int wpl;
+  int epoch;
 };
 
 template <bool MULTI = false>
@@ -812,6 +818,97 @@
   rhs[kN + 1] = u.y;
 }
 
+template <typename TIN, typename TOUT, bool BWD, bool MULTI, bool TR>
+__device__ __forceinline__ void settle_group(const Problem &p, const WinSet &ws, const Args &a, const int g, const unsigned long long m,
+                                             const int timed_out, const int lane) {
+  const int b = TR ? g * a.sm.tr_u : g / a.ndg, dg = TR ? 0 : g - b * a.ndg;
+  const int d0 = dg * a.dgw;
+  const int sd_all = MULTI ? a.sm.total : p.sd;
+  const int nd = TR ? (a.sm.tr_B - b < a.sm.tr_u ? a.sm.tr_B - b : a.sm.tr_u) * a.sm.tr_nd
+                    : (sd_all - d0 < a.dgw ? sd_all - d0 : a.dgw);
+  if (lane >= nd || !((m >> lane) & 1ull)) return;
+  int d = d0 + lane, dstat = d;
+  const int Tmax = p.Tmax;
+  int T = p.lengths ? p.lengths[TR ? b + d / a.sm.tr_nd : b] : Tmax;
+  T = T < 0 ? 0 : (T > Tmax ? Tmax : T);
+  int status = -1;
+  if (MULTI) {
+    const StreamMap &smk = a.sm;
+    LaneStream ls;
+    if (TR) {
+      ls = lane_stream_tr(a.sm, d);
+    } else {
+      const int s_ = (d >= smk.begin[1]) + (d >= smk.begin[2]) + (d >= smk.begin[3]);
+      const int dl = d - smk.begin[s_];
+      ls = {smk.sd[s_], dl + smk.in_col[s_], dl + smk.stat_col[s_], dl + smk.out_col[s_], dl + smk.in_col[s_]};
+    }
+    Problem q = p;
+    q.sd = ls.sd;
+    q.D = ws.nw * ls.sd;
+    q.mean = (const TIN *)p.mean + ls.din;
+    q.var = p.var ? (const void *)((const TIN *)p.var + (p.var_mode == MLPG_HIP_VAR_GLOBAL ? ls.dvar : ls.din)) : nullptr;
+    if (!timed_out) {
+      const SysView<TIN, BWD> view = make_view<TIN, BWD>(q, ws, b, 0, T);
+      status = first_bad_pivot<2, TIN, BWD>(view, ws);
+      if (status == 0) status = -2;
+    }
+    dstat = ls.dstat;
+    d = ls.dout;
+  } else if (!timed_out) {
+    const SysView<TIN, BWD> view = make_view<TIN, BWD>(p, ws, b, d, T);
+    status = first_bad_pivot<2, TIN, BWD>(view, ws);
+    if (status == 0) status = -2;
+  }
+  if (p.status) p.status[(size_t)b * p.ld_status + dstat] = status;
+  TOUT *out_b = (TOUT *)p.out + (size_t)b * Tmax * p.ld_out;
+  for (int t = 0; t < Tmax; ++t) {
+    if (!BWD) out_b[(size_t)t * p.ld_out + d] = (TOUT)0;
+    else
+      for (int w = 0; w < ws.nw; ++w) out_b[(size_t)t * p.ld_out + w * p.sd + d] = (TOUT)0;
+  }
+}
+template <typename TIN, typename TOUT, bool BWD, bool MULTI, bool TR>
+__device__ __forceinline__ void settle_marked(const Problem &p, const WinSet &ws, const Args &a, const int wv, const int lane) {
+  for (int g0 = 0; g0 < a.nsg; g0 += 64) {
+    int *line = a.ctrl + (size_t)(1 + kMaxLists + g0 + lane) * kCtrlLine;
+    int m_lo = 0, m_hi = 0, to = 0;
+    if (g0 + lane < a.nsg) {
+      m_lo = __hip_atomic_load(line + 2, __ATOMIC_RELAXED, __HIP_MEMORY_SCOPE_AGENT);
+      m_hi = __hip_atomic_load(line + 3, __ATOMIC_RELAXED, __HIP_MEMORY_SCOPE_AGENT);
+      to = __hip_atomic_load(line + 4, __ATOMIC_RELAXED, __HIP_MEMORY_SCOPE_AGENT);
+    }
+    const bool mine = (m_lo | m_hi | to) != 0 && ((g0 + lane) % kW) == wv;
+    unsigned long long todo = __ballot(mine);
+    while (todo != 0ull) {
+      const int k = __builtin_ctzll(todo);
+      todo &= todo - 1ull;
+      const unsigned long long m = (unsigned long long)(unsigned)__shfl(m_lo, k, 64) | ((unsigned long long)(unsigned)__shfl(m_hi, k, 64) << 32);
+      settle_group<TIN, TOUT, BWD, MULTI, TR>(p, ws, a, g0 + k, m, __shfl(to, k, 64), lane);
+    }
+    if (mine) {
+      __hip_atomic_store(line + 2, 0, __ATOMIC_RELAXED, __HIP_MEMORY_SCOPE_AGENT);
+      __hip_atomic_store(line + 3, 0, __ATOMIC_RELAXED, __HIP_MEMORY_SCOPE_AGENT);
+      __hip_atomic_store(line + 4, 0, __ATOMIC_RELAXED, __HIP_MEMORY_SCOPE_AGENT);
+    }
+  }
+}
+
+__device__ __forceinline__ int flags_set(const int *first, const int n, const int lane, const int epoch) {
+  int ln = lane;
+  asm volatile("" : "+v"(ln));
+  const int *fp = first + ln;
+  int f = 1;
+#pragma unroll
+  for (int k = 0; k < 4; ++k) {
+    if (k * 64 < n) {
+      int v = epoch;
+      if (ln < n - k * 64) v = __hip_atomic_load(fp + k * 64, __ATOMIC_RELAXED, __HIP_MEMORY_SCOPE_AGENT);
+      f &= v == epoch;
+    }
+  }
+  return f;
+}
+
 template <typename TIN, typename TOUT, bool BWD, int VM, bool MULTI = false, bool NW3 = true, bool TR = false, bool STD = false>
 __global__ __launch_bounds__(kW * 64, MLPG_STRIP_WGS) void strip_kernel(Problem p, WinSet ws, Args a) {
   static_assert(!TR || MULTI, "the transposed form is a MULTI kernel");
@@ -1034,7 +1131,10 @@
       int *line = a.ctrl + (1 + kMaxLists + g) * kCtrlLine;
       __hip_atomic_fetch_or(line + 2, (int)(unsigned)m, __ATOMIC_RELAXED, __HIP_MEMORY_SCOPE_AGENT);
       __hip_atomic_fetch_or(line + 3, (int)(unsigned)(m >> 32), __ATOMIC_RELAXED, __HIP_MEMORY_SCOPE_AGENT);
-      if (to) __hip_atomic_store(line + 4, 1, __ATOMIC_RELAXED, __HIP_MEMORY_SCOPE_AGENT);
+      int one = 1, bit = kDoneMarked;
+      asm volatile("" : "+v"(one), "+v"(bit));
+      if (to) __hip_atomic_store(line + 4, one, __ATOMIC_RELAXED, __HIP_MEMORY_SCOPE_AGENT);
+      if (MLPG_STRIP_SETTLE_INLINE) __hip_atomic_fetch_or(a.ctrl + kDoneWord, bit, __ATOMIC_RELAXED, __HIP_MEMORY_SCOPE_AGENT);
     }
 #if !defined(MLPG_STRIP_TIMING) && !defined(MLPG_STRIP_TRACE)
     if (r == 0 && lane_ok && p.status) p.status[(size_t)b * p.ld_status + dstat] = 0;
@@ -1283,19 +1383,17 @@
       }
       asm volatile("s_waitcnt vmcnt(0)" ::: "memory");
       STRIP_TICK(5);
-      int *cnt = a.ctrl + (1 + kMaxLists + g) * kCtrlLine;
       int *flags = a.ctrl + (1 + kMaxLists + a.nsg) * kCtrlLine + (size_t)g * flag_pitch(R);
       if (lane == 0) {
-        __hip_atomic_fetch_add(cnt, 1, __ATOMIC_RELAXED, __HIP_MEMORY_SCOPE_AGENT);
-        __hip_atomic_store(flags + r, 1, __ATOMIC_RELAXED, __HIP_MEMORY_SCOPE_AGENT);
+        int ep = a.epoch;
+        asm volatile("" : "+s"(ep));
+        __hip_atomic_store(flags + r, ep, __ATOMIC_RELAXED, __HIP_MEMORY_SCOPE_AGENT);
       }
       {
         const Window w = local_window(r, Ract, kwin);
         int spins = 0, ok = 1;
         for (;;) {
-          int f = 1;
-          if (route == 0) f = __hip_atomic_load(cnt, __ATOMIC_RELAXED, __HIP_MEMORY_SCOPE_AGENT) >= Ract;
-          else if (lane <= w.hiE - w.lo) f = __hip_atomic_load(flags + w.lo + lane, __ATOMIC_RELAXED, __HIP_MEMORY_SCOPE_AGENT);
+          const int f = route == 0 ? flags_set(flags, Ract, lane, a.epoch) : flags_set(flags + w.lo, w.hiE - w.lo + 1, lane, a.epoch);
           if (__ballot(f == 0) == 0ull) break;
           __builtin_amdgcn_s_sleep(MLPG_STRIP_POLL_SLEEP);
           if (++spins > kSpinLimit) { ok = 0; break; }
@@ -1424,7 +1522,6 @@
         sweep(0, Ract - 1, 0);
       } else {
         int cur = route;
-        int *cnt = a.ctrl + (1 + kMaxLists + g) * kCtrlLine;
         int *flags = a.ctrl + (1 + kMaxLists + a.nsg) * kCtrlLine + (size_t)g * flag_pitch(R);
         for (;;) {
           const Window w = local_window(r, Ract, cur);
@@ -1439,15 +1536,13 @@
             const Window w2 = local_window(r, Ract, kLocal);
             int spins = 0;
             for (;;) {
-              int f = 1;
-              if (lane <= w2.hiE - w2.lo) f = __hip_atomic_load(flags + w2.lo + lane, __ATOMIC_RELAXED, __HIP_MEMORY_SCOPE_AGENT);
-              if (__ballot(f == 0) == 0ull) break;
+              if (__ballot(!flags_set(flags + w2.lo, w2.hiE - w2.lo + 1, lane, a.epoch)) == 0ull) break;
               __builtin_amdgcn_s_sleep(MLPG_STRIP_POLL_SLEEP);
               if (++spins > kSpinLimit) { ok = 0; break; }
             }
           } else if (next == 2) {
             int spins = 0;
-            while (__hip_atomic_load(cnt, __ATOMIC_RELAXED, __HIP_MEMORY_SCOPE_AGENT) < Ract) {
+            while (__ballot(!flags_set(flags, Ract, lane, a.epoch)) != 0ull) {
               __builtin_amdgcn_s_sleep(32);
               if (++spins > kSpinLimit) { ok = 0; break; }
             }
@@ -1577,7 +1672,9 @@
     for (;;) {
       if (tid == 0) {
         int tk = lim;
-        if (__hip_atomic_load(ticket, __ATOMIC_RELAXED, __HIP_MEMORY_SCOPE_AGENT) < lim) tk = atomicAdd(ticket, 1);
+        int one = 1;
+        asm volatile("" : "+v"(one));
+        if (__hip_atomic_load(ticket, __ATOMIC_RELAXED, __HIP_MEMORY_SCOPE_AGENT) < lim) tk = atomicAdd(ticket, one);
         if (first_item && a.stagger > 0 && tk < a.wpl && tk < lim) {
           const long long until = t_launch + (long long)tk * a.stagger / a.wpl;
           while ((long long)__builtin_amdgcn_s_memrealtime() < until) __builtin_amdgcn_s_sleep(8);
@@ -1599,8 +1696,37 @@
     }
     __syncthreads();
   }
-}
-
+
+#if MLPG_STRIP_SETTLE_INLINE
+  asm volatile("s_waitcnt vmcnt(0)" ::: "memory");
+  __syncthreads();
+  if (tid == 0) {
+    __builtin_amdgcn_fence(__ATOMIC_RELEASE, "agent");
+    asm volatile("s_waitcnt vmcnt(0)" ::: "memory");
+    int one = 1;
+    asm volatile("" : "+v"(one));
+    lds_misc[4] = __hip_atomic_fetch_add(a.ctrl + kDoneWord, one, __ATOMIC_RELAXED, __HIP_MEMORY_SCOPE_AGENT);
+  }
+  __syncthreads();
+  const int done = __builtin_amdgcn_readfirstlane(lds_misc[4]);
+  if ((done & (kDoneMarked - 1)) != (int)gridDim.x - 1) return;
+  if (tid == 0) {
+    __builtin_amdgcn_fence(__ATOMIC_ACQUIRE, "agent");
+    asm volatile("s_waitcnt vmcnt(0)" ::: "memory");
+  }
+  __syncthreads();
+  for (int i = tid; i < (1 + kMaxLists) * kCtrlLine; i += kW * 64) __hip_atomic_store(a.ctrl + i, 0, __ATOMIC_RELAXED, __HIP_MEMORY_SCOPE_AGENT);
+  if (done & kDoneMarked) {
+    const unsigned long long kp = (unsigned long long)__builtin_amdgcn_kernarg_segment_ptr();
+    unsigned kl = (unsigned)kp, kh = (unsigned)(kp >> 32);
+    asm volatile("" : "+v"(kl), "+v"(kh));
+    const char *kb = (const char *)(((unsigned long long)kh << 32) | kl);
+    settle_marked<TIN, TOUT, BWD, MULTI, TR>(*(const Problem *)kb, *(const WinSet *)(kb + kKargWs), *(const Args *)(kb + kKargArgs), wv, lane);
+  }
+#endif
+}
+
+#if !MLPG_STRIP_SETTLE_INLINE
 template <typename TIN, typename TOUT, bool BWD, bool MULTI = false, bool TR = false>
 __global__ void __launch_bounds__(256) verdict_kernel(const Problem p, const WinSet ws, const Args a) {
   const int lane = threadIdx.x & 63;
@@ -1610,49 +1736,17 @@
   const unsigned long long m = (unsigned long long)(unsigned)line[2] | ((unsigned long long)(unsigned)line[3] << 32);
   const int timed_out = line[4];
   __builtin_amdgcn_wave_barrier();
-  if (lane < 5) line[lane] = 0;
-  for (int i = lane; i < flag_pitch(a.R); i += 64) a.ctrl[(1 + kMaxLists + a.nsg) * kCtrlLine + (size_t)g * flag_pitch(a.R) + i] = 0;
+  if (lane >= 2 && lane < 5 && (m != 0ull || timed_out)) line[lane] = 0;
   if (g == 0)
     for (int i = lane; i < (1 + kMaxLists) * kCtrlLine; i += 64) a.ctrl[i] = 0;
   if (m == 0ull) return;
-  const int b = TR ? g * a.sm.tr_u : g / a.ndg, dg = TR ? 0 : g - b * a.ndg;
-  const int d0 = dg * a.dgw;
-  const int sd_all = MULTI ? a.sm.total : p.sd;
-  const int nd = TR ? (a.sm.tr_B - b < a.sm.tr_u ? a.sm.tr_B - b : a.sm.tr_u) * a.sm.tr_nd
-                    : (sd_all - d0 < a.dgw ? sd_all - d0 : a.dgw);
-  if (lane >= nd || !((m >> lane) & 1ull)) return;
-  int d = d0 + lane, dstat = d;
-  const int Tmax = p.Tmax;
-  int T = p.lengths ? p.lengths[TR ? b + d / a.sm.tr_nd : b] : Tmax;
-  T = T < 0 ? 0 : (T > Tmax ? Tmax : T);
-  int status = -1;
-  if (MULTI) {
-    const LaneStream ls = TR ? lane_stream_tr(a.sm, d) : lane_stream(a.sm, d);
-    Problem q = p;
-    q.sd = ls.sd;
-    q.D = ws.nw * ls.sd;
-    q.mean = (const TIN *)p.mean + ls.din;
-    q.var = p.var ? (const void *)((const TIN *)p.var + (p.var_mode == MLPG_HIP_VAR_GLOBAL ? ls.dvar : ls.din)) : nullptr;
-    if (!timed_out) {
-      const SysView<TIN, BWD> view = make_view<TIN, BWD>(q, ws, b, 0, T);
-      status = first_bad_pivot<2, TIN, BWD>(view, ws);
-      if (status == 0) status = -2;
-    }
-    dstat = ls.dstat;
-    d = ls.dout;
-  } else if (!timed_out) {
-    const SysView<TIN, BWD> view = make_view<TIN, BWD>(p, ws, b, d, T);
-    status = first_bad_pivot<2, TIN, BWD>(view, ws);
-    if (status == 0) status = -2;
-  }
-  if (p.status) p.status[(size_t)b * p.ld_status + dstat] = status;
-  TOUT *out_b = (TOUT *)p.out + (size_t)b * Tmax * p.ld_out;
-  for (int t = 0; t < Tmax; ++t) {
-    if (!BWD) out_b[(size_t)t * p.ld_out + d] = (TOUT)0;
-    else
-      for (int w = 0; w < ws.nw; ++w) out_b[(size_t)t * p.ld_out + w * p.sd + d] = (TOUT)0;
-  }
-}
+  const unsigned long long kp = (unsigned long long)__builtin_amdgcn_kernarg_segment_ptr();
+  unsigned kl = (unsigned)kp, kh = (unsigned)(kp >> 32);
+  asm volatile("" : "+v"(kl), "+v"(kh));
+  const char *kb = (const char *)(((unsigned long long)kh << 32) | kl);
+  settle_group<TIN, TOUT, BWD, MULTI, TR>(*(const Problem *)kb, *(const WinSet *)(kb + kKargWs), *(const Args *)(kb + kKargArgs), g, m, timed_out, lane);
+}
+#endif
 
 inline size_t ctrl_bytes(int nsg, int R) { return (ctrl_ints(nsg, R) * sizeof(int) + 255) / 256 * 256; }
 
@@ -1698,7 +1792,7 @@
 
 template <typename TIN, typename TOUT, bool BWD, bool MULTI, bool TR = false>
 int launch_impl(hipStream_t st, const Problem &p, const WinSet &ws, void *scratch_base, int R, int ndg, int dgw,
-                bool zero_ctrl, const StreamMap *smap) {
+                bool zero_ctrl, int epoch, const StreamMap *smap) {
   Args a;
   memset(&a.sm, 0, sizeof(a.sm));
   if (MULTI) a.sm = *smap;
@@ -1710,6 +1804,7 @@
   a.dgw = dgw;
   a.nsg = nsg;
   a.one = 1.0;
+  a.epoch = epoch;
   for (int w = 0; w < ws.nw; ++w) {
     const int l = ws.l[w], u = ws.u[w];
     const double *cw = ws.c + ws.off[w];
@@ -1746,8 +1841,10 @@
     note_launch(TR ? kCountStripTr : MULTI ? kCountStripMulti : kCountStrip);
     hipLaunchKernelGGL(kern, dim3((unsigned)grid), dim3(kW * 64), kLdsBytes, st, p, ws, a);
     MLPG_HIP_CHECK(hipGetLastError());
+#if !MLPG_STRIP_SETTLE_INLINE
     hipLaunchKernelGGL((verdict_kernel<TIN, TOUT, BWD, MULTI, TR>), dim3((unsigned)((nsg + 3) / 4)), dim3(256), 0, st, p, ws, a);
     MLPG_HIP_CHECK(hipGetLastError());
+#endif
     return 0;
   };
   if constexpr (MULTI) {
@@ -1777,18 +1874,18 @@
 
 template <typename TIN, typename TOUT, bool BWD>
 int launch_t(hipStream_t st, const Problem &p, const WinSet &ws, void *scratch_base, int R, int ndg, int dgw,
-             bool zero_ctrl) {
-  return launch_impl<TIN, TOUT, BWD, false>(st, p, ws, scratch_base, R, ndg, dgw, zero_ctrl, nullptr);
+             bool zero_ctrl, int epoch) {
+  return launch_impl<TIN, TOUT, BWD, false>(st, p, ws, scratch_base, R, ndg, dgw, zero_ctrl, epoch, nullptr);
 }
 template <typename TIN, typename TOUT>
 int launch_multi_t(hipStream_t st, const Problem &p, const WinSet &ws, void *scratch_base, int R, int ndg, int dgw,
-                   bool zero_ctrl, const StreamMap &smap) {
-  return launch_impl<TIN, TOUT, false, true>(st, p, ws, scratch_base, R, ndg, dgw, zero_ctrl, &smap);
+                   bool zero_ctrl, int epoch, const StreamMap &smap) {
+  return launch_impl<TIN, TOUT, false, true>(st, p, ws, scratch_base, R, ndg, dgw, zero_ctrl, epoch, &smap);
 }
 template <typename TIN, typename TOUT>
-int launch_tr_t(hipStream_t st, const Problem &p, const WinSet &ws, void *scratch_base, int R, bool zero_ctrl, const StreamMap &smap) {
-  return launch_impl<TIN, TOUT, false, true, true>(st, p, ws, scratch_base, R, 1, 64, zero_ctrl, &smap);
-}
-
-}
-}
+int launch_tr_t(hipStream_t st, const Problem &p, const WinSet &ws, void *scratch_base, int R, bool zero_ctrl, int epoch, const StreamMap &smap) {
+  return launch_impl<TIN, TOUT, false, true, true>(st, p, ws, scratch_base, R, 1, 64, zero_ctrl, epoch, &smap);
+}
+
+}
+}
diff --git a/nnmnkwii_amd/csrc/mlpg_strip_multi_f32.hip b/nnmnkwii_amd/csrc/mlpg_strip_multi_f32.hip
--- a/nnmnkwii_amd/csrc/mlpg_strip_multi_f32.hip
+++ b/nnmnkwii_amd/csrc/mlpg_strip_multi_f32.hip
@@ -1,9 +1,9 @@
 #include "mlpg_strip_impl.h"
 namespace mlpg {
-int launch_strip_multi_f32(hipStream_t st, const Problem &p, const WinSet &ws, void *scratch, int R, int ndg, int dgw, bool zero_ctrl, const StreamMap &sm) {
-  return strip::launch_multi_t<float, float>(st, p, ws, scratch, R, ndg, dgw, zero_ctrl, sm);
+int launch_strip_multi_f32(hipStream_t st, const Problem &p, const WinSet &ws, void *scratch, int R, int ndg, int dgw, bool zero_ctrl, int epoch, const StreamMap &sm) {
+  return strip::launch_multi_t<float, float>(st, p, ws, scratch, R, ndg, dgw, zero_ctrl, epoch, sm);
 }
-int launch_strip_tr_f32(hipStream_t st, const Problem &p, const WinSet &ws, void *scratch, int R, bool zero_ctrl, const StreamMap &sm) {
-  return strip::launch_tr_t<float, float>(st, p, ws, scratch, R, zero_ctrl, sm);
+int launch_strip_tr_f32(hipStream_t st, const Problem &p, const WinSet &ws, void *scratch, int R, bool zero_ctrl, int epoch, const StreamMap &sm) {
+  return strip::launch_tr_t<float, float>(st, p, ws, scratch, R, zero_ctrl, epoch, sm);
 }
 }
diff --git a/nnmnkwii_amd/csrc/mlpg_strip_multi_f64.hip b/nnmnkwii_amd/csrc/mlpg_strip_multi_f64.hip
--- a/nnmnkwii_amd/csrc/mlpg_strip_multi_f64.hip
+++ b/nnmnkwii_amd/csrc/mlpg_strip_multi_f64.hip
@@ -1,9 +1,9 @@
 #include "mlpg_strip_impl.h"
 namespace mlpg {
-int launch_strip_multi_f64(hipStream_t st, const Problem &p, const WinSet &ws, void *scratch, int R, int ndg, int dgw, bool zero_ctrl, const StreamMap &sm) {
-  return strip::launch_multi_t<double, double>(st, p, ws, scratch, R, ndg, dgw, zero_ctrl, sm);
+int launch_strip_multi_f64(hipStream_t st, const Problem &p, const WinSet &ws, void *scratch, int R, int ndg, int dgw, bool zero_ctrl, int epoch, const StreamMap &sm) {
+  return strip::launch_multi_t<double, double>(st, p, ws, scratch, R, ndg, dgw, zero_ctrl, epoch, sm);
 }
-int launch_strip_tr_f64(hipStream_t st, const Problem &p, const WinSet &ws, void *scratch, int R, bool zero_ctrl, const StreamMap &sm) {
-  return strip::launch_tr_t<double, double>(st, p, ws, scratch, R, zero_ctrl, sm);
+int launch_strip_tr_f64(hipStream_t st, const Problem &p, const WinSet &ws, void *scratch, int R, bool zero_ctrl, int epoch, const StreamMap &sm) {
+  return strip::launch_tr_t<double, double>(st, p, ws, scratch, R, zero_ctrl, epoch, sm);
 }
 }
```

After: 1.280 billion. No clear change (-0.3%).
